# NickTravers/NeuralNetworkLibrary

Measured on AMD Instinct MI355X. Metric: ResNet-34 224x224 training throughput (Learner.train1minibatch, fwd+loss+bwd+optimizer), higher is better.
Workload: dtype f32; 1 GPU; DogsCats ResNet-34 classifier, 224x224, bs=64 per GPU, SGD momentum 0.9, fp32; global_batch=64, image_size=224, parallelism=dp1

## Files before the change

### include/nnl.h

```cpp
#ifndef NNL_H_
#define NNL_H_

#include <stddef.h>
#include <stdint.h>

#ifdef __cplusplus
extern "C" {
#endif

typedef enum {
  NNL_OK = 0,
  NNL_ERR_INVALID_ARG = -1,
  NNL_ERR_HIP = -2,
  NNL_ERR_UNSUPPORTED = -3,
  NNL_ERR_WORKSPACE = -4
} nnl_status_t;

int nnl_version(void);
const char* nnl_last_error(void);
int nnl_reload_env(void);

enum { NNL_PROF_CONV_FWD = 0, NNL_PROF_CONV_DGRAD = 1, NNL_PROF_CONV_WGRAD = 2, NNL_PROF_EMBDOT = 3,
       NNL_PROF_TABULAR = 4, NNL_PROF_RETINA_LOSS = 5, NNL_PROF_LSTM = 6, NNL_PROF_SOFTMAX_CE = 7,
       NNL_PROF_ELEMENTWISE = 8, NNL_PROF_GEMM = 9, NNL_PROF_OPTIM = 10, NNL_PROF_KINDS = 11 };
int nnl_prof_enable(int enable);
int nnl_prof_collect(int64_t* launches, double* total_ms, double* total_work);
int nnl_prof_collect2(int64_t* launches, double* total_ms, double* total_work, double* total_exec);
int nnl_dp_bump(int32_t* step, void* stream);
int nnl_dp_signal(int32_t* flag, const int32_t* step, void* stream);
int nnl_dp_wait(const int32_t* flag, int32_t value, int64_t timeout_us, int32_t* err, void* stream);
const char* nnl_source_stamp(void);

int nnl_embdotbias_fwd(const int64_t* x, const float* U, const float* M, const float* bu, const float* bi,
                       float* y, float* z, int64_t n, int64_t n_user, int64_t n_item, int64_t D,
                       int has_range, float lo, float hi, int32_t* err_flag, void* stream);
size_t nnl_embdotbias_bwd_workspace_bytes(int64_t n);
int nnl_embdotbias_bwd(const int64_t* x, const float* U, const float* M, const float* z, const float* dy,
                       float* dU, float* dM, float* dbu, float* dbi, int64_t n, int64_t n_user,
                       int64_t n_item, int64_t D, int has_range, float lo, float hi, void* workspace, size_t workspace_bytes, void* stream);

typedef struct {
  int32_t N, H, W, C;
  int32_t K, R, S;
  int32_t stride, pad;
  int32_t P, Q;
} nnl_conv_geom_t;

size_t nnl_conv2d_fwd_workspace_bytes(const nnl_conv_geom_t* g);
int64_t nnl_conv2d_tile_counters(void);
int nnl_conv2d_fwd(const float* x, const float* w, const float* bias, float* y, const nnl_conv_geom_t* g,
                   int relu, void* workspace, size_t workspace_bytes, int32_t* tile_counters, float* bn_partials,
                   const float* bn_pivot, int32_t* bn_rows, void* stream);
int nnl_conv2d_fwd_add_up2(const float* x, const float* w, const float* bias, const float* small, float* y,
                           const nnl_conv_geom_t* g, void* stream);
int nnl_upsample2_bwd(const float* dy, float* dsmall, int64_t N, int64_t h, int64_t w, int64_t C, void* stream);
int nnl_conv2d_weight_transpose(const float* w, float* wt, int K, int R, int S, int C, void* stream);
typedef struct {
  const float* w;
  float* wt;
  int32_t K, RS, C, first_tile;
} nnl_wt_desc_t;
int nnl_conv2d_weight_transpose_multi(const nnl_wt_desc_t* desc, const int32_t* tile_tensor, int64_t n_tiles,
                                      double total_elems, void* stream);
size_t nnl_conv2d_dgrad_workspace_bytes(const nnl_conv_geom_t* g);
int nnl_conv2d_dgrad(const float* dy, const float* wt, float* dx, const nnl_conv_geom_t* g, const float* addend,
                     void* workspace, size_t workspace_bytes, int32_t* tile_counters, void* stream);
typedef struct {
  const float* src;
  float* dst;
  int32_t rows, ch, flip, first_block;
  int32_t two_d, reserved;
} nnl_wino_desc_t;
int nnl_conv2d_wino_preferred(const nnl_conv_geom_t* g, int dgrad);
int nnl_wino_filter_multi(const nnl_wino_desc_t* desc, const int32_t* block_desc, int64_t n_blocks, void* stream);
int nnl_conv2d_fwd_pre(const float* x, const float* w, const float* bias, float* y, const nnl_conv_geom_t* g, int relu,
                       void* workspace, size_t workspace_bytes, int32_t* tile_counters, float* bn_partials, const float* bn_pivot,
                       int32_t* bn_rows, const float* u, void* stream);
int nnl_conv2d_dgrad_pre(const float* dy, const float* wt, float* dx, const nnl_conv_geom_t* g, const float* addend,
                         void* workspace, size_t workspace_bytes, int32_t* tile_counters, const float* u, void* stream);
size_t nnl_debug_conv_wino_workspace_bytes(int N, int H, int W, int C, int K);
int nnl_debug_conv_wino_fwd(const float* x, const float* filt, const float* bias, const float* add, float* y, void* ws,
                            size_t ws_bytes, int32_t* counters, long n_counters, float* bn_part, const float* bn_pivot, int N,
                            int H, int W, int C, int K, int relu, int flip, void* stream);
size_t nnl_debug_conv_wino2_workspace_bytes(int N, int H, int W, int C, int K);
int nnl_debug_conv_wino2_fwd(const float* x, const float* filt, const float* bias, const float* add, float* y, void* ws,
                            size_t ws_bytes, int32_t* counters, long n_counters, float* bn_part, const float* bn_pivot, int N,
                            int H, int W, int C, int K, int relu, int flip, void* stream);
int nnl_debug_conv_plan_times(int N, int H, int W, int C, int K, double* out);

int nnl_debug_route_record(int enable);
int nnl_debug_route_collect(char* out, size_t n);
size_t nnl_conv2d_wgrad_workspace_bytes(const nnl_conv_geom_t* g);
int nnl_conv2d_wgrad(const float* x, const float* dy, float* dw, const nnl_conv_geom_t* g, void* workspace,
                     size_t workspace_bytes, void* stream);
size_t nnl_colsum_workspace_bytes(int64_t rows, int64_t cols);
int nnl_sum_tensors(const float* const* src, int n, float* out, int64_t numel, void* stream);
int nnl_colsum(const float* a, float* out, int64_t rows, int64_t cols, void* workspace, size_t workspace_bytes,
               void* stream);
int nnl_relu_gate_colsum(const float* dy, const float* y, float* g, float* colsum, int64_t rows, int64_t cols, void* workspace,
                         size_t workspace_bytes, void* stream);
int nnl_act_gate_colsum(const float* dy, const float* y, float* g, float* colsum, int64_t rows, int64_t cols, int act,
                        void* workspace, size_t workspace_bytes, void* stream);

size_t nnl_bn_workspace_bytes(int64_t rows, int64_t C);
int nnl_bn_fwd(const float* x, const float* gamma, const float* beta, const float* residual, float* y,
               float* save_mean, float* save_invstd, float* running_mean, float* running_var, int64_t rows,
               int64_t C, float eps, float momentum, int training, int relu, int64_t* num_batches_tracked,
               uint32_t* relu_mask, const float* ext_partials, int64_t ext_rows, const float* ext_pivot, float* pivot_out,
               void* workspace, size_t workspace_bytes, void* stream);
int nnl_bn_bwd(const float* dy, const float* y, const uint32_t* relu_mask, const float* x, const float* gamma,
               const float* mean, const float* invstd, float* dx, float* dres, float* dgamma, float* dbeta, int64_t rows,
               int64_t C, int training, int relu, void* workspace, size_t workspace_bytes, void* stream);

int nnl_bn_relu_maxpool_supported(int64_t C);
int nnl_bn_relu_maxpool_fwd(const float* x, const float* gamma, const float* beta, float* y, uint8_t* idx, float* save_mean,
                            float* save_invstd, float* save_scale, float* save_shift, float* running_mean, float* running_var,
                            int64_t N, int64_t H, int64_t W, int64_t C, int64_t P, int64_t Q, int ks, int stride, int pad, float eps,
                            float momentum, int training, int64_t* num_batches_tracked, void* workspace, size_t workspace_bytes,
                            void* stream);
int nnl_bn_relu_maxpool_bwd(const float* dpool, const float* y, const uint8_t* idx, const float* x, const float* gamma,
                            const float* beta, const float* mean, const float* invstd, const float* scale, const float* shift,
                            float* dx, float* dgamma, float* dbeta,
                            int64_t N, int64_t H, int64_t W, int64_t C, int64_t P, int64_t Q, int ks, int stride, int pad,
                            int training, void* workspace, size_t workspace_bytes, void* stream);

int nnl_bn_sync_stats(const float* x, float* stats, int64_t rows, int64_t C, void* workspace, size_t workspace_bytes,
                      void* stream);
int nnl_bn_sync_fwd(const float* x, const float* all_stats, int world, const float* gamma, const float* beta,
                    const float* residual, float* y, float* save_mean, float* save_invstd, float* running_mean,
                    float* running_var, int64_t rows, int64_t C, float eps, float momentum, int relu,
                    int64_t* num_batches_tracked, uint32_t* relu_mask, void* workspace, size_t workspace_bytes, void* stream);
int nnl_bn_sync_bwd_reduce(const float* dy, const float* y, const uint32_t* relu_mask, const float* x, const float* mean,
                           const float* invstd, float* sums, int64_t rows, int64_t C, int relu, void* workspace,
                           size_t workspace_bytes, void* stream);
int nnl_bn_sync_bwd(const float* dy, const float* y, const uint32_t* relu_mask, const float* x, const float* gamma,
                    const float* mean, const float* invstd, const float* local_sums, const float* global_sums,
                    const float* all_stats,
                    int world, float* dx, float* dres, float* dgamma, float* dbeta, int64_t rows, int64_t C, int relu,
                    void* workspace, size_t workspace_bytes, void* stream);

int nnl_maxpool2d_fwd(const float* x, float* y, uint8_t* idx, int64_t N, int64_t H, int64_t W, int64_t C, int64_t P,
                      int64_t Q, int ksize, int stride, int pad, void* stream);
int nnl_maxpool2d_bwd(const float* dy, const uint8_t* idx, float* dx, int64_t N, int64_t H, int64_t W, int64_t C,
                      int64_t P, int64_t Q, int ksize, int stride, int pad, void* stream);
int nnl_concat_pool_fwd(const float* x, float* out, int32_t* argmax, int64_t N, int64_t HW, int64_t C, void* stream);
int nnl_concat_pool_bwd(const float* dout, const int32_t* argmax, float* dx, int64_t N, int64_t HW, int64_t C, void* stream);

int nnl_bbox_decode(const float* anchors, const float* reg, const float* clas, int64_t bs, int64_t A, int64_t K,
                    const float* mean4, const float* std4, float thresh, float width, float height, float* cand_boxes,
                    int32_t* cand_classes, float* cand_scores, int32_t* cand_order, int32_t* cand_count, void* stream);
size_t nnl_nms_workspace_bytes(int64_t bs, int64_t top_k);
int nnl_nms(const float* cand_boxes, const int32_t* cand_classes, const float* cand_scores, const int32_t* cand_order,
            const int32_t* cand_count, int64_t bs, int64_t cap, int64_t top_k, float max_overlap, float* kept_boxes,
            int32_t* kept_classes, float* kept_scores, int32_t* kept_count, void* workspace, size_t workspace_bytes,
            void* stream);

int nnl_tab_renorm(const int64_t* xcat, float* const* tables, const int32_t* card, const int32_t* dim,
                   const int32_t* row_off, const int32_t* row_table, int32_t* flags, int64_t bs, int32_t ncat,
                   int32_t total_rows, float max_norm, int32_t* err_flag, void* stream);
int nnl_tab_gather_fwd(const int64_t* xcat, const float* const* tables, const int32_t* card, const int32_t* dim,
                       const int32_t* col_off, const int32_t* col_table, const float* row_mask, const float* cont,
                       const float* cont_mask, float* out, int64_t bs, int32_t ncat, int32_t cat_width,
                       int32_t n_cont, int32_t ld_out, void* stream);
size_t nnl_tab_scatter_bwd_workspace_bytes(int64_t bs, int32_t ncat);
int nnl_tab_scatter_bwd(const int64_t* xcat, const int32_t* card, const int32_t* dim, const int32_t* col_off,
                        const int32_t* col_table, const int64_t* grad_off, const float* row_mask,
                        const float* cont_mask, const float* dout, float* dtab_flat, int64_t dtab_elems,
                        float* dcont, int64_t bs, int32_t ncat, int32_t cat_width, int32_t n_cont, int32_t ld_out,
                        void* workspace, size_t workspace_bytes, void* stream);
int nnl_tab_scan_bwd(const int64_t* xcat, const int32_t* card, const int32_t* dim, const int32_t* col_off,
                     const int64_t* grad_off, const float* row_mask, const float* cont_mask, const float* dout,
                     float* dtab_flat, float* dcont, const int32_t* blk_col, const int32_t* blk_first, int32_t n_scan_blocks,
                     int32_t max_dim, int64_t bs, int32_t ncat, int32_t cat_width, int32_t n_cont, int32_t ld_out, void* stream);

int nnl_pad_cols(const float* src, float* dst, int64_t rows, int64_t C, int64_t Cp, void* stream);
int nnl_keep_masks(const float* u, float* a, int64_t na, float keep_a, float* b, int64_t nb, float keep_b, void* stream);

int nnl_linear_small_supported(int64_t N);
int nnl_linear_small_fwd(const float* x, const float* w, const float* bias, float* y, int64_t M, int64_t K, int64_t ldx, int64_t N,
                         void* stream);
size_t nnl_linear_small_bwd_workspace_bytes(int64_t M, int64_t K, int64_t N);
int nnl_linear_small_bwd(const float* dy, const float* x, const float* w, float* dx, float* dw, float* db, int64_t M, int64_t K,
                         int64_t ldx, int64_t N, void* workspace, size_t workspace_bytes, void* stream);

size_t nnl_retina_loss_workspace_bytes(int64_t bs, int64_t A);
int nnl_retina_loss_fwd(const float* anchors, const float* reg, const float* clas, const float* boxes,
                        const int64_t* cats, int32_t* state, float* npos, float* out, int64_t bs, int64_t A,
                        int64_t K, int64_t M, float beta, float alpha, float gamma, void* workspace,
                        size_t workspace_bytes, void* stream);
int nnl_retina_loss_bwd(const float* anchors, const float* reg, const float* clas, const float* boxes,
                        const int64_t* cats, const int32_t* state, const float* npos, const float* grad_out,
                        float* dreg, float* dclas, int64_t bs, int64_t A, int64_t K, int64_t M, float beta,
                        float alpha, float gamma, void* stream);

int64_t nnl_lstm_padded_hidden(int64_t H);
int64_t nnl_lstm_padded_gates(int64_t H);
size_t nnl_lstm_workspace_bytes(int64_t T, int64_t B, int64_t H);
int nnl_lstm_fwd(const float* gx, const float* w_hh_pad, const float* h0, const float* c0, float* y, float* cy,
                 float* gates, int64_t T, int64_t B, int64_t H, void* workspace, size_t workspace_bytes, int32_t* err_flag,
                 void* stream);
int nnl_lstm_bwd(const float* dy, const float* dhT, const float* dcT, const float* gates, const float* cy,
                 const float* c0, const float* w_hh_t_pad, float* dgates_pad, float* dh0, float* dc0, int64_t T, int64_t B,
                 int64_t H, void* workspace, size_t workspace_bytes, int32_t* err_flag, void* stream);
int nnl_debug_lstm_bptt2_plan(int64_t B, int64_t H, int32_t* out5);

size_t nnl_mse_workspace_bytes(int64_t n);
int nnl_mse_fwd(const float* pred, const float* target, float* loss, int64_t n, void* workspace, size_t workspace_bytes, void* stream);
int nnl_mse_bwd(const float* pred, const float* target, const float* grad_out, float* dpred, int64_t n, void* stream);
int nnl_scaled_sigmoid_fwd(const float* x, float* y, float* sig, int64_t n, float lo, float hi, void* stream);
int nnl_scaled_sigmoid_bwd(const float* dy, const float* sig, float* dx, int64_t n, float lo, float hi, void* stream);

int nnl_embedding_rowmask_fwd(const int64_t* x, const float* W, const float* rowmask, float* out, int64_t n,
                              int64_t V, int64_t D, int32_t* err_flag, void* stream);
size_t nnl_embedding_rowmask_bwd_workspace_bytes(int64_t n);
int nnl_embedding_rowmask_bwd(const int64_t* x, const float* rowmask, const float* dout, float* dW, int64_t n,
                              int64_t V, int64_t D, int64_t padding_idx, void* workspace, size_t workspace_bytes, void* stream);
int nnl_softmax_ce_fwd(const float* logits, const int64_t* target, float* lse, float* loss_rows, float* loss_mean,
                       int64_t rows, int64_t V, int32_t* err_flag, void* stream);
int nnl_softmax_ce_bwd(const float* logits, const int64_t* target, const float* lse, const float* grad_out,
                       float* dlogits, int64_t rows, int64_t V, int64_t ld_dlogits, void* stream);
size_t nnl_seq_reg_workspace_bytes(int64_t T, int64_t R);
int nnl_seq_reg_fwd(const float* h, float* out3, int64_t T, int64_t R, float alpha, float beta, void* workspace,
                    size_t workspace_bytes, void* stream);
int nnl_seq_reg_bwd(const float* h, const float* grad_out, float* dh, int64_t T, int64_t R, float alpha, float beta, void* stream);
int nnl_weight_drop(const float* src, int64_t ld_src, const float* mask, float* out, int64_t ld_out, int64_t rows, int64_t H,
                    uint64_t seed, float p, void* stream);

size_t nnl_attn_pool_workspace_bytes(int64_t T, int64_t B, int64_t E, int64_t A);
int nnl_attn_pool_fwd(const float* h, const float* w2, const float* b2, const float* enc_out, const int64_t* x, int64_t pad_token,
                      float* attn, float* pooled, int64_t T, int64_t B, int64_t E, int64_t A, void* workspace, size_t workspace_bytes,
                      int32_t* counters, int64_t n_counters, void* stream);
int nnl_attn_pool_bwd(const float* h, const float* w2, const float* enc_out, const float* attn, const float* dpooled,
                      const float* dattn, float* dh, float* denc, float* dw2, float* db2, int64_t T, int64_t B, int64_t E, int64_t A,
                      void* workspace, size_t workspace_bytes, int32_t* counters, int64_t n_counters, void* stream);

typedef struct {
  float* param;
  float* grad;
  float* state1;
  float* state2;
  int64_t numel;
  float lr;
  float decay;
} nnl_optim_tensor_t;
int64_t nnl_optim_chunk_elems(void);
int nnl_optim_patch(nnl_optim_tensor_t* tensors, float* hyper, const float* dyn, int64_t n, void* stream);
int nnl_optim_step(const nnl_optim_tensor_t* tensors, const int32_t* chunk_tensor, const int64_t* chunk_off,
                   int64_t n_chunks, int kind, const float* hyper, int use_clip, float* clip_workspace, void* stream);

#ifdef __cplusplus
}
#endif
#endif
```

### neuralnetworklibrary_amd/_lib.py

```python
import ctypes as C
import os

import torch

_HERE = os.path.dirname(os.path.abspath(__file__))
LIB_PATH = os.environ.get('NNL_LIB_PATH') or os.path.join(_HERE, 'libnnl_hip.so')

if not os.path.exists(LIB_PATH):
    raise ImportError(
        f"{LIB_PATH} not found: build it with `python -c 'import __graft_entry__ as g; g.build()'` "
        "(or `make -C neuralnetworklibrary_amd/csrc`). There is no CPU fallback for the HIP hot path.")

lib = C.CDLL(LIB_PATH)

c_p = C.c_void_p
i32, i64, f32, f64 = C.c_int32, C.c_int64, C.c_float, C.c_double
sz = C.c_size_t


class ConvGeom(C.Structure):
    _fields_ = [('N', i32), ('H', i32), ('W', i32), ('C', i32), ('K', i32), ('R', i32), ('S', i32),
                ('stride', i32), ('pad', i32), ('P', i32), ('Q', i32)]


SIGNATURES = {
    'nnl_version': (C.c_int, []),
    'nnl_last_error': (C.c_char_p, []),
    'nnl_reload_env': (C.c_int, []),
    'nnl_prof_enable': (C.c_int, [C.c_int]),
    'nnl_prof_collect': (C.c_int, [C.POINTER(i64), C.POINTER(f64), C.POINTER(f64)]),
    'nnl_prof_collect2': (C.c_int, [C.POINTER(i64), C.POINTER(f64), C.POINTER(f64), C.POINTER(f64)]),
    'nnl_source_stamp': (C.c_char_p, []),
    'nnl_dp_bump': (C.c_int, [c_p, c_p]),
    'nnl_dp_signal': (C.c_int, [c_p, c_p, c_p]),
    'nnl_dp_wait': (C.c_int, [c_p, i32, i64, c_p, c_p]),
    'nnl_embdotbias_fwd': (C.c_int, [c_p, c_p, c_p, c_p, c_p, c_p, c_p, i64, i64, i64, i64, C.c_int, f32, f32,
                                     c_p, c_p]),
    'nnl_embdotbias_bwd_workspace_bytes': (sz, [i64]),
    'nnl_embdotbias_bwd': (C.c_int, [c_p, c_p, c_p, c_p, c_p, c_p, c_p, c_p, c_p, i64, i64, i64, i64, C.c_int,
                                     f32, f32, c_p, sz, c_p]),
    'nnl_conv2d_fwd_workspace_bytes': (sz, [C.POINTER(ConvGeom)]),
    'nnl_conv2d_dgrad_workspace_bytes': (sz, [C.POINTER(ConvGeom)]),
    'nnl_conv2d_tile_counters': (i64, []),
    'nnl_conv2d_wino_preferred': (C.c_int, [C.POINTER(ConvGeom), C.c_int]),
    'nnl_wino_filter_multi': (C.c_int, [c_p, c_p, i64, c_p]),
    'nnl_conv2d_fwd_pre': (C.c_int, [c_p, c_p, c_p, c_p, C.POINTER(ConvGeom), C.c_int, c_p, sz, c_p, c_p, c_p, C.POINTER(i32), c_p, c_p]),
    'nnl_conv2d_dgrad_pre': (C.c_int, [c_p, c_p, c_p, C.POINTER(ConvGeom), c_p, c_p, sz, c_p, c_p, c_p]),
    'nnl_debug_conv_wino_workspace_bytes': (sz, [C.c_int] * 5),
    'nnl_debug_conv_wino_fwd': (C.c_int, [c_p] * 6 + [sz, c_p, C.c_long, c_p, c_p] + [C.c_int] * 7 + [c_p]),
    'nnl_debug_conv_wino2_workspace_bytes': (sz, [C.c_int] * 5),
    'nnl_debug_conv_wino2_fwd': (C.c_int, [c_p] * 6 + [sz, c_p, C.c_long, c_p, c_p] + [C.c_int] * 7 + [c_p]),
    'nnl_debug_conv_plan_times': (C.c_int, [C.c_int] * 5 + [C.POINTER(C.c_double)]),
    'nnl_debug_route_record': (C.c_int, [C.c_int]),
    'nnl_debug_route_collect': (C.c_int, [C.c_char_p, sz]),
    'nnl_conv2d_fwd': (C.c_int, [c_p, c_p, c_p, c_p, C.POINTER(ConvGeom), C.c_int, c_p, sz, c_p, c_p, c_p, C.POINTER(i32), c_p]),
    'nnl_conv2d_weight_transpose': (C.c_int, [c_p, c_p, C.c_int, C.c_int, C.c_int, C.c_int, c_p]),
    'nnl_conv2d_weight_transpose_multi': (C.c_int, [c_p, c_p, i64, f64, c_p]),
    'nnl_conv2d_dgrad': (C.c_int, [c_p, c_p, c_p, C.POINTER(ConvGeom), c_p, c_p, sz, c_p, c_p]),
    'nnl_conv2d_wgrad_workspace_bytes': (sz, [C.POINTER(ConvGeom)]),
    'nnl_conv2d_wgrad': (C.c_int, [c_p, c_p, c_p, C.POINTER(ConvGeom), c_p, sz, c_p]),
    'nnl_colsum_workspace_bytes': (sz, [i64, i64]),
    'nnl_colsum': (C.c_int, [c_p, c_p, i64, i64, c_p, sz, c_p]),
    'nnl_relu_gate_colsum': (C.c_int, [c_p, c_p, c_p, c_p, i64, i64, c_p, sz, c_p]),
    'nnl_conv2d_fwd_add_up2': (C.c_int, [c_p, c_p, c_p, c_p, c_p, C.POINTER(ConvGeom), c_p]),
    'nnl_upsample2_bwd': (C.c_int, [c_p, c_p, i64, i64, i64, i64, c_p]),
    'nnl_act_gate_colsum': (C.c_int, [c_p, c_p, c_p, c_p, i64, i64, C.c_int, c_p, sz, c_p]),
    'nnl_maxpool2d_fwd': (C.c_int, [c_p, c_p, c_p, i64, i64, i64, i64, i64, i64, C.c_int, C.c_int, C.c_int, c_p]),
    'nnl_maxpool2d_bwd': (C.c_int, [c_p, c_p, c_p, i64, i64, i64, i64, i64, i64, C.c_int, C.c_int, C.c_int, c_p]),
    'nnl_sum_tensors': (C.c_int, [c_p, C.c_int, c_p, i64, c_p]),
    'nnl_bn_relu_maxpool_supported': (C.c_int, [i64]),
    'nnl_bn_relu_maxpool_fwd': (C.c_int, [c_p, c_p, c_p, c_p, c_p, c_p, c_p, c_p, c_p, c_p, c_p, i64, i64, i64, i64, i64, i64,
                                          C.c_int, C.c_int, C.c_int, f32, f32, C.c_int, c_p, c_p, sz, c_p]),
    'nnl_bn_relu_maxpool_bwd': (C.c_int, [c_p, c_p, c_p, c_p, c_p, c_p, c_p, c_p, c_p, c_p, c_p, c_p, c_p, i64, i64, i64, i64, i64, i64,
                                          C.c_int, C.c_int, C.c_int, C.c_int, c_p, sz, c_p]),
    'nnl_concat_pool_fwd': (C.c_int, [c_p, c_p, c_p, i64, i64, i64, c_p]),
    'nnl_concat_pool_bwd': (C.c_int, [c_p, c_p, c_p, i64, i64, i64, c_p]),
    'nnl_bbox_decode': (C.c_int, [c_p, c_p, c_p, i64, i64, i64, c_p, c_p, f32, f32, f32, c_p, c_p, c_p, c_p, c_p, c_p]),
    'nnl_nms_workspace_bytes': (sz, [i64, i64]),
    'nnl_nms': (C.c_int, [c_p, c_p, c_p, c_p, c_p, i64, i64, i64, f32, c_p, c_p, c_p, c_p, c_p, sz, c_p]),
    'nnl_tab_renorm': (C.c_int, [c_p, c_p, c_p, c_p, c_p, c_p, c_p, i64, i32, i32, f32, c_p, c_p]),
    'nnl_tab_gather_fwd': (C.c_int, [c_p, c_p, c_p, c_p, c_p, c_p, c_p, c_p, c_p, c_p, i64, i32, i32, i32, i32, c_p]),
    'nnl_tab_scatter_bwd_workspace_bytes': (sz, [i64, i32]),
    'nnl_tab_scatter_bwd': (C.c_int, [c_p, c_p, c_p, c_p, c_p, c_p, c_p, c_p, c_p, c_p, i64, c_p, i64, i32, i32, i32, i32, c_p, sz, c_p]),
    'nnl_tab_scan_bwd': (C.c_int, [c_p] * 12 + [i32, i32, i64, i32, i32, i32, i32, c_p]),
    'nnl_pad_cols': (C.c_int, [c_p, c_p, i64, i64, i64, c_p]),
    'nnl_keep_masks': (C.c_int, [c_p, c_p, i64, f32, c_p, i64, f32, c_p]),
    'nnl_linear_small_supported': (C.c_int, [i64]),
    'nnl_linear_small_fwd': (C.c_int, [c_p, c_p, c_p, c_p, i64, i64, i64, i64, c_p]),
    'nnl_linear_small_bwd_workspace_bytes': (sz, [i64, i64, i64]),
    'nnl_linear_small_bwd': (C.c_int, [c_p, c_p, c_p, c_p, c_p, c_p, i64, i64, i64, i64, c_p, sz, c_p]),
    'nnl_retina_loss_workspace_bytes': (sz, [i64, i64]),
    'nnl_retina_loss_fwd': (C.c_int, [c_p, c_p, c_p, c_p, c_p, c_p, c_p, c_p, i64, i64, i64, i64, f32, f32, f32, c_p, sz, c_p]),
    'nnl_retina_loss_bwd': (C.c_int, [c_p, c_p, c_p, c_p, c_p, c_p, c_p, c_p, c_p, c_p, i64, i64, i64, i64, f32, f32, f32, c_p]),
    'nnl_lstm_padded_hidden': (i64, [i64]),
    'nnl_lstm_padded_gates': (i64, [i64]),
    'nnl_lstm_workspace_bytes': (sz, [i64, i64, i64]),
    'nnl_lstm_fwd': (C.c_int, [c_p, c_p, c_p, c_p, c_p, c_p, c_p, i64, i64, i64, c_p, sz, c_p, c_p]),
    'nnl_lstm_bwd': (C.c_int, [c_p, c_p, c_p, c_p, c_p, c_p, c_p, c_p, c_p, c_p, i64, i64, i64, c_p, sz, c_p, c_p]),
    'nnl_debug_lstm_bptt2_plan': (C.c_int, [i64, i64, c_p]),
    'nnl_embedding_rowmask_fwd': (C.c_int, [c_p, c_p, c_p, c_p, i64, i64, i64, c_p, c_p]),
    'nnl_embedding_rowmask_bwd_workspace_bytes': (sz, [i64]),
    'nnl_embedding_rowmask_bwd': (C.c_int, [c_p, c_p, c_p, c_p, i64, i64, i64, i64, c_p, sz, c_p]),
    'nnl_softmax_ce_fwd': (C.c_int, [c_p, c_p, c_p, c_p, c_p, i64, i64, c_p, c_p]),
    'nnl_softmax_ce_bwd': (C.c_int, [c_p, c_p, c_p, c_p, c_p, i64, i64, i64, c_p]),
    'nnl_mse_workspace_bytes': (sz, [i64]),
    'nnl_mse_fwd': (C.c_int, [c_p, c_p, c_p, i64, c_p, sz, c_p]),
    'nnl_mse_bwd': (C.c_int, [c_p, c_p, c_p, c_p, i64, c_p]),
    'nnl_scaled_sigmoid_fwd': (C.c_int, [c_p, c_p, c_p, i64, C.c_float, C.c_float, c_p]),
    'nnl_scaled_sigmoid_bwd': (C.c_int, [c_p, c_p, c_p, i64, C.c_float, C.c_float, c_p]),
    'nnl_seq_reg_workspace_bytes': (sz, [i64, i64]),
    'nnl_seq_reg_fwd': (C.c_int, [c_p, c_p, i64, i64, C.c_float, C.c_float, c_p, sz, c_p]),
    'nnl_seq_reg_bwd': (C.c_int, [c_p, c_p, c_p, i64, i64, C.c_float, C.c_float, c_p]),
    'nnl_weight_drop': (C.c_int, [c_p, i64, c_p, c_p, i64, i64, i64, C.c_uint64, C.c_float, c_p]),
    'nnl_attn_pool_workspace_bytes': (sz, [i64, i64, i64, i64]),
    'nnl_attn_pool_fwd': (C.c_int, [c_p, c_p, c_p, c_p, c_p, i64, c_p, c_p, i64, i64, i64, i64, c_p, sz, c_p, i64, c_p]),
    'nnl_attn_pool_bwd': (C.c_int, [c_p, c_p, c_p, c_p, c_p, c_p, c_p, c_p, c_p, c_p, i64, i64, i64, i64, c_p, sz, c_p, i64, c_p]),
    'nnl_optim_chunk_elems': (i64, []),
    'nnl_optim_patch': (C.c_int, [c_p, c_p, c_p, i64, c_p]),
    'nnl_optim_step': (C.c_int, [c_p, c_p, c_p, i64, C.c_int, c_p, C.c_int, c_p, c_p]),
    'nnl_bn_workspace_bytes': (sz, [i64, i64]),
    'nnl_bn_fwd': (C.c_int, [c_p, c_p, c_p, c_p, c_p, c_p, c_p, c_p, c_p, i64, i64, f32, f32, C.c_int, C.c_int, c_p, c_p, c_p, i64,
                             c_p, c_p, c_p, sz, c_p]),
    'nnl_bn_sync_stats': (C.c_int, [c_p, c_p, i64, i64, c_p, sz, c_p]),
    'nnl_bn_sync_fwd': (C.c_int, [c_p, c_p, C.c_int, c_p, c_p, c_p, c_p, c_p, c_p, c_p, c_p, i64, i64, f32, f32, C.c_int, c_p,
                                  c_p, c_p, sz, c_p]),
    'nnl_bn_sync_bwd_reduce': (C.c_int, [c_p, c_p, c_p, c_p, c_p, c_p, c_p, i64, i64, C.c_int, c_p, sz, c_p]),
    'nnl_bn_sync_bwd': (C.c_int, [c_p, c_p, c_p, c_p, c_p, c_p, c_p, c_p, c_p, c_p, C.c_int, c_p, c_p, c_p, c_p, i64, i64,
                                  C.c_int, c_p, sz, c_p]),
    'nnl_bn_bwd': (C.c_int, [c_p, c_p, c_p, c_p, c_p, c_p, c_p, c_p, c_p, c_p, c_p, i64, i64, C.c_int, C.c_int, c_p, sz, c_p]),
}

for _name, (_res, _args) in SIGNATURES.items():
    try:
        _fn = getattr(lib, _name)
    except AttributeError as e:
        raise ImportError(f"libnnl_hip.so does not export {_name}; rebuild it") from e
    _fn.restype = _res
    _fn.argtypes = _args

PROF_KINDS = ['conv_fwd', 'conv_dgrad', 'conv_wgrad', 'embdot', 'tabular', 'retina_loss', 'lstm',
              'softmax_ce', 'elementwise', 'gemm', 'optim']


class NnlError(RuntimeError):
    pass


def check(status):
    if status != 0:
        raise NnlError(f"nnl error {status}: {lib.nnl_last_error().decode()}")


def ptr(t):
    return None if t is None else C.c_void_p(t.data_ptr())


def stream():
    return C.c_void_p(torch.cuda.current_stream().cuda_stream)


def require_cuda(*tensors):
    for t in tensors:
        if t is not None and not t.is_cuda:
            raise NnlError("nnl HIP op called with a non-CUDA tensor: the MI355X path has no CPU fallback")


def prof_enable(flag=True):
    check(lib.nnl_prof_enable(1 if flag else 0))


def prof_collect():
    n = len(PROF_KINDS)
    a, b, c, d = (i64 * n)(), (f64 * n)(), (f64 * n)(), (f64 * n)()
    check(lib.nnl_prof_collect2(a, b, c, d))
    return {k: {'launches': int(a[i]), 'ms': float(b[i]), 'work': float(c[i]), 'exec': float(d[i])} for i, k in enumerate(PROF_KINDS)}


def source_stamp_of_tree():
    import glob
    import hashlib
    csrc = os.path.join(os.path.dirname(os.path.abspath(__file__)), 'csrc')
    names = sorted(os.path.basename(p) for p in glob.glob(os.path.join(csrc, '*.hip')) + glob.glob(os.path.join(csrc, '*.h')))
    hsh = hashlib.sha256()
    for p in [os.path.join(csrc, n) for n in names] + [os.path.join(csrc, 'Makefile'), os.path.join(csrc, '..', '..', 'include', 'nnl.h')]:
        with open(p, 'rb') as f:
            hsh.update(f.read())
    return hsh.hexdigest()[:16]


def source_stamp():
    return lib.nnl_source_stamp().decode()
```

### neuralnetworklibrary_amd/csrc/batchnorm.hip

```cpp
#include "nnl_common.h"

namespace {

typedef float f32x4 __attribute__((ext_vector_type(4)));

template <int VEC> struct VecT;
template <> struct VecT<4> { typedef f32x4 type; };
template <> struct VecT<1> { typedef float type; };

template <int VEC> __device__ __forceinline__ float vget(const typename VecT<VEC>::type& v, int i);
template <> __device__ __forceinline__ float vget<4>(const f32x4& v, int i) { return v[i]; }
template <> __device__ __forceinline__ float vget<1>(const float& v, int i) { return v; }
template <int VEC> __device__ __forceinline__ void vset(typename VecT<VEC>::type& v, int i, float x);
template <> __device__ __forceinline__ void vset<4>(f32x4& v, int i, float x) { v[i] = x; }
template <> __device__ __forceinline__ void vset<1>(float& v, int i, float x) { v = x; }

constexpr int kBlock = 256;
constexpr int kMaxRowBlocks = 1024;
constexpr int kFinLanes = 64;

struct Shape {
  int L;
  int rpb;
  int gx, gy;
};

Shape make_shape(long rows, long CG) {
  Shape s;
  s.L = 1;
  while (s.L < 64 && s.L < CG) s.L <<= 1;
  s.rpb = kBlock / s.L;
  s.gy = (int)nnl_cdiv(CG, s.L);
  long gx = nnl_cdiv(rows, (long)s.rpb * 4);
  long cap = kMaxRowBlocks / (s.gy > 0 ? s.gy : 1);
  if (cap < 1) cap = 1;
  if (gx > cap) gx = cap;
  if (gx < 1) gx = 1;
  s.gx = (int)gx;
  return s;
}

template <int VEC>
__global__ __launch_bounds__(kBlock) void bn_stats_kernel(const float* __restrict__ x, float* __restrict__ part,
                                                           long rows, int C, int L) {
  typedef typename VecT<VEC>::type V;
  __shared__ float red[kBlock * 2 * VEC];
  const int CG = C / VEC;
  const int tx = threadIdx.x & (L - 1), ty = threadIdx.x / L;
  const int rpb = kBlock / L;
  const int g = blockIdx.y * L + tx;
  const bool ok = g < CG;
  float s1[VEC], s2[VEC], piv[VEC];
#pragma unroll
  for (int e = 0; e < VEC; ++e) { s1[e] = 0.f; s2[e] = 0.f; piv[e] = 0.f; }
  if (ok) {
    const V pv = *reinterpret_cast<const V*>(x + (long)g * VEC);
#pragma unroll
    for (int e = 0; e < VEC; ++e) piv[e] = vget<VEC>(pv, e);
    const long rstep = (long)gridDim.x * rpb;
    long r = (long)blockIdx.x * rpb + ty;
    const float* xp = x + (long)g * VEC;
    for (; r + 3 * rstep < rows; r += 4 * rstep) {
      V v[4];
#pragma unroll
      for (int u = 0; u < 4; ++u) v[u] = *reinterpret_cast<const V*>(xp + (r + u * rstep) * C);
#pragma unroll
      for (int u = 0; u < 4; ++u)
#pragma unroll
        for (int e = 0; e < VEC; ++e) {
          const float d = vget<VEC>(v[u], e) - piv[e];
          s1[e] += d;
          s2[e] += d * d;
        }
    }
    for (; r < rows; r += rstep) {
      const V v = *reinterpret_cast<const V*>(xp + r * C);
#pragma unroll
      for (int e = 0; e < VEC; ++e) {
        const float d = vget<VEC>(v, e) - piv[e];
        s1[e] += d;
        s2[e] += d * d;
      }
    }
  }
#pragma unroll
  for (int e = 0; e < VEC; ++e) {
    red[(threadIdx.x * VEC + e) * 2 + 0] = s1[e];
    red[(threadIdx.x * VEC + e) * 2 + 1] = s2[e];
  }
  __syncthreads();
  if (ty == 0 && ok) {
#pragma unroll
    for (int e = 0; e < VEC; ++e) {
      float a = 0.f, b = 0.f;
      for (int j = 0; j < rpb; ++j) {
        a += red[((j * L + tx) * VEC + e) * 2 + 0];
        b += red[((j * L + tx) * VEC + e) * 2 + 1];
      }
      const long c = (long)g * VEC + e;
      part[((long)blockIdx.x * C + c) * 2 + 0] = a;
      part[((long)blockIdx.x * C + c) * 2 + 1] = b;
    }
  }
}

template <int LANES = kFinLanes>
__device__ __forceinline__ void reduce_partials(const float* __restrict__ part, int nparts, int C, int c, bool cok,
                                                float (*red)[LANES][2], float& s1, float& s2) {
  const int lane = threadIdx.x & (LANES - 1), ch = threadIdx.x / LANES;
  float a = 0.f, b = 0.f;
  if (cok) {
    typedef float f32x2 __attribute__((ext_vector_type(2)));
    const f32x2* pp = reinterpret_cast<const f32x2*>(part) + c;
    int p = lane;
    constexpr int U = 8;
    for (; p + (U - 1) * LANES < nparts; p += U * LANES) {
      f32x2 v[U];
#pragma unroll
      for (int u = 0; u < U; ++u) v[u] = pp[(long)(p + u * LANES) * C];
#pragma unroll
      for (int u = 0; u < U; ++u) { a += v[u][0]; b += v[u][1]; }
    }
    for (; p < nparts; p += LANES) {
      const f32x2 v = pp[(long)p * C];
      a += v[0]; b += v[1];
    }
  }
  red[ch][lane][0] = a;
  red[ch][lane][1] = b;
  __syncthreads();
  for (int w = LANES / 2; w > 0; w >>= 1) {
    if (lane < w) {
      red[ch][lane][0] += red[ch][lane + w][0];
      red[ch][lane][1] += red[ch][lane + w][1];
    }
    __syncthreads();
  }
  s1 = red[ch][0][0];
  s2 = red[ch][0][1];
}

__device__ __forceinline__ void finish_stats(int c, int C, float m, float var, float n, const float* __restrict__ gamma,
                                             const float* __restrict__ beta, float* __restrict__ mean,
                                             float* __restrict__ invstd, float* __restrict__ running_mean,
                                             float* __restrict__ running_var, float* __restrict__ scale,
                                             float* __restrict__ shift, float eps, float momentum,
                                             float* __restrict__ pivot_out = nullptr) {
  const float is = 1.f / sqrtf(var + eps);
  mean[c] = m;
  if (pivot_out) pivot_out[c] = m;
  invstd[c] = is;
  if (running_mean) running_mean[c] = (1.f - momentum) * running_mean[c] + momentum * m;
  if (running_var) {
    const float unbiased = n > 1.f ? var * (n / (n - 1.f)) : var;
    running_var[c] = (1.f - momentum) * running_var[c] + momentum * unbiased;
  }
  const float gm = gamma ? gamma[c] : 1.f;
  const float sc = is * gm;
  scale[c] = sc;
  shift[c] = (beta ? beta[c] : 0.f) - m * sc;
}

template <int LANES>
__global__ void bn_finalize_kernel(const float* __restrict__ x, const float* __restrict__ part, int nparts,
                                   const float* __restrict__ gamma, const float* __restrict__ beta,
                                   float* __restrict__ mean, float* __restrict__ invstd,
                                   float* __restrict__ running_mean, float* __restrict__ running_var,
                                   float* __restrict__ scale, float* __restrict__ shift, long rows, int C, float eps,
                                   float momentum, long long* __restrict__ num_batches_tracked,
                                   float* __restrict__ pivot_out) {
  __shared__ float red[256 / LANES][LANES][2];
  const int c = blockIdx.x * (256 / LANES) + threadIdx.x / LANES;
  float s1, s2;
  reduce_partials<LANES>(part, nparts, C, c, c < C, red, s1, s2);
  if (c >= C || (threadIdx.x & (LANES - 1)) != 0) return;
  if (c == 0 && num_batches_tracked) *num_batches_tracked += 1;
  const float n = (float)rows;
  const float m = x[c] + s1 / n;
  float var = (s2 - s1 * (s1 / n)) / n;
  var = fmaxf(var, 0.f);
  finish_stats(c, C, m, var, n, gamma, beta, mean, invstd, running_mean, running_var, scale, shift, eps, momentum, pivot_out);
}

__global__ void bn_sync_local_kernel(const float* __restrict__ x, const float* __restrict__ part, int nparts,
                                     float* __restrict__ stats, long rows, int C) {
  __shared__ float red[4][kFinLanes][2];
  const int c = blockIdx.x * 4 + threadIdx.x / kFinLanes;
  float s1, s2;
  reduce_partials(part, nparts, C, c, c < C, red, s1, s2);
  if (c >= C || (threadIdx.x & (kFinLanes - 1)) != 0) return;
  const float n = (float)rows;
  stats[c] = x[c] + s1 / n;
  stats[C + c] = fmaxf(s2 - s1 * (s1 / n), 0.f);
  if (c == 0) {
    stats[2 * C] = (float)(rows >> 16);
    stats[2 * C + 1] = (float)(rows & 0xFFFF);
  }
}

__device__ __forceinline__ float sync_count(const float* __restrict__ st, int C) { return st[2 * C] * 65536.f + st[2 * C + 1]; }

__global__ void bn_sync_merge_kernel(const float* __restrict__ all_stats, int world, const float* __restrict__ gamma,
                                     const float* __restrict__ beta, float* __restrict__ mean, float* __restrict__ invstd,
                                     float* __restrict__ running_mean, float* __restrict__ running_var,
                                     float* __restrict__ scale, float* __restrict__ shift, int C, float eps, float momentum,
                                     long long* __restrict__ num_batches_tracked) {
  const int c = blockIdx.x * blockDim.x + threadIdx.x;
  if (c >= C) return;
  if (c == 0 && num_batches_tracked) *num_batches_tracked += 1;
  const long stride = 2L * C + 2;
  float n = 0.f, m = 0.f, M2 = 0.f;
  for (int r = 0; r < world; ++r) {
    const float* st = all_stats + r * stride;
    const float nr = sync_count(st, C);
    if (nr <= 0.f) continue;
    const float nn = n + nr;
    const float d = st[c] - m;
    m += d * (nr / nn);
    M2 += st[C + c] + d * d * (n * (nr / nn));
    n = nn;
  }
  finish_stats(c, C, m, fmaxf(M2 / n, 0.f), n, gamma, beta, mean, invstd, running_mean, running_var, scale, shift, eps, momentum);
}

__global__ void bn_eval_scale_kernel(const float* __restrict__ gamma, const float* __restrict__ beta,
                                     const float* __restrict__ running_mean, const float* __restrict__ running_var,
                                     float* __restrict__ scale, float* __restrict__ shift, float* __restrict__ invstd,
                                     int C, float eps) {
  const int c = blockIdx.x * blockDim.x + threadIdx.x;
  if (c >= C) return;
  const float is = 1.f / sqrtf(running_var[c] + eps);
  const float sc = is * (gamma ? gamma[c] : 1.f);
  scale[c] = sc;
  shift[c] = (beta ? beta[c] : 0.f) - running_mean[c] * sc;
  if (invstd) invstd[c] = is;
}

template <int VEC>
__device__ __forceinline__ unsigned keep_bits(const unsigned* __restrict__ mask, long i) {
  const long bit = i * VEC;
  return (mask[bit >> 5] >> (bit & 31)) & ((1u << VEC) - 1u);
}

template <int VEC>
__global__ __launch_bounds__(kBlock) void bn_apply_kernel(const float* __restrict__ x, const float* __restrict__ scale,
                                                           const float* __restrict__ shift,
                                                           const float* __restrict__ residual, float* __restrict__ y,
                                                           long total_v, int CG, int relu, unsigned* __restrict__ mask) {
  typedef typename VecT<VEC>::type V;
  const long stride = (long)gridDim.x * blockDim.x;
  const long i0 = (long)blockIdx.x * blockDim.x + threadIdx.x;
  const int lane = threadIdx.x & 63;
  const int g = (int)((unsigned long)i0 % (unsigned)CG);
  const V sc = reinterpret_cast<const V*>(scale)[g];
  const V sh = reinterpret_cast<const V*>(shift)[g];
  for (long base = i0 - lane; base < total_v; base += stride) {
    const long i = base + lane;
    const bool ok = i < total_v;
    unsigned bits = 0;
    if (ok) {
      const V xv = reinterpret_cast<const V*>(x)[i];
      V out;
      if (residual) {
        const V rv = reinterpret_cast<const V*>(residual)[i];
#pragma unroll
        for (int e = 0; e < VEC; ++e) vset<VEC>(out, e, vget<VEC>(xv, e) * vget<VEC>(sc, e) + vget<VEC>(sh, e) + vget<VEC>(rv, e));
      } else {
#pragma unroll
        for (int e = 0; e < VEC; ++e) vset<VEC>(out, e, vget<VEC>(xv, e) * vget<VEC>(sc, e) + vget<VEC>(sh, e));
      }
      if (relu) {
#pragma unroll
        for (int e = 0; e < VEC; ++e) {
          if (vget<VEC>(out, e) > 0.f) bits |= 1u << e;
          vset<VEC>(out, e, fmaxf(vget<VEC>(out, e), 0.f));
        }
      }
      reinterpret_cast<V*>(y)[i] = out;
    }
    if (mask != nullptr) {
      if (VEC == 4) {
        unsigned w = bits << ((lane & 7) * 4);
        w |= __shfl_xor(w, 1, 64);
        w |= __shfl_xor(w, 2, 64);
        w |= __shfl_xor(w, 4, 64);
        if ((lane & 7) == 0 && ok) mask[i >> 3] = w;
      } else {
        const unsigned long long b = __ballot(bits & 1u);
        if (lane == 0 && ok) mask[base >> 5] = (unsigned)b;
        if (lane == 32 && ok) mask[(base >> 5) + 1] = (unsigned)(b >> 32);
      }
    }
  }
}

template <int VEC>
__global__ __launch_bounds__(kBlock) void bn_bwd_reduce_kernel(const float* __restrict__ dy, const float* __restrict__ y,
                                                                const float* __restrict__ x, const float* __restrict__ mean,
                                                                const float* __restrict__ invstd, float* __restrict__ part,
                                                                long rows, int C, int L, int relu,
                                                                const unsigned* __restrict__ mask) {
  typedef typename VecT<VEC>::type V;
  __shared__ float red[kBlock * 2 * VEC];
  const int CG = C / VEC;
  const int tx = threadIdx.x & (L - 1), ty = threadIdx.x / L;
  const int rpb = kBlock / L;
  const int g = blockIdx.y * L + tx;
  const bool ok = g < CG;
  float s1[VEC], s2[VEC], mu[VEC], is[VEC];
#pragma unroll
  for (int e = 0; e < VEC; ++e) { s1[e] = 0.f; s2[e] = 0.f; mu[e] = 0.f; is[e] = 0.f; }
  if (ok) {
#pragma unroll
    for (int e = 0; e < VEC; ++e) { mu[e] = mean[(long)g * VEC + e]; is[e] = invstd[(long)g * VEC + e]; }
    const long rstep = (long)gridDim.x * rpb;
    long r = (long)blockIdx.x * rpb + ty;
    for (; r + rstep < rows; r += 2 * rstep) {
      V dv[2], xv[2], yv[2];
      unsigned kb[2] = {~0u, ~0u};
#pragma unroll
      for (int u = 0; u < 2; ++u) {
        const long off = (r + u * rstep) * C + (long)g * VEC;
        dv[u] = *reinterpret_cast<const V*>(dy + off);
        xv[u] = *reinterpret_cast<const V*>(x + off);
        yv[u] = dv[u];
        if (relu) {
          if (mask) kb[u] = keep_bits<VEC>(mask, off / VEC);
          else yv[u] = *reinterpret_cast<const V*>(y + off);
        }
      }
#pragma unroll
      for (int u = 0; u < 2; ++u)
#pragma unroll
        for (int e = 0; e < VEC; ++e) {
          float gg = vget<VEC>(dv[u], e);
          if (relu && (mask ? !((kb[u] >> e) & 1u) : !(vget<VEC>(yv[u], e) > 0.f))) gg = 0.f;
          s1[e] += gg;
          s2[e] += gg * ((vget<VEC>(xv[u], e) - mu[e]) * is[e]);
        }
    }
    for (; r < rows; r += rstep) {
      const long off = r * C + (long)g * VEC;
      const V dv = *reinterpret_cast<const V*>(dy + off);
      const V xv = *reinterpret_cast<const V*>(x + off);
      V yv = dv;
      unsigned kb = ~0u;
      if (relu) {
        if (mask) kb = keep_bits<VEC>(mask, off / VEC);
        else yv = *reinterpret_cast<const V*>(y + off);
      }
#pragma unroll
      for (int e = 0; e < VEC; ++e) {
        float gg = vget<VEC>(dv, e);
        if (relu && (mask ? !((kb >> e) & 1u) : !(vget<VEC>(yv, e) > 0.f))) gg = 0.f;
        s1[e] += gg;
        s2[e] += gg * ((vget<VEC>(xv, e) - mu[e]) * is[e]);
      }
    }
  }
#pragma unroll
  for (int e = 0; e < VEC; ++e) {
    red[(threadIdx.x * VEC + e) * 2 + 0] = s1[e];
    red[(threadIdx.x * VEC + e) * 2 + 1] = s2[e];
  }
  __syncthreads();
  if (ty == 0 && ok) {
#pragma unroll
    for (int e = 0; e < VEC; ++e) {
      float a = 0.f, b = 0.f;
      for (int j = 0; j < rpb; ++j) {
        a += red[((j * L + tx) * VEC + e) * 2 + 0];
        b += red[((j * L + tx) * VEC + e) * 2 + 1];
      }
      const long c = (long)g * VEC + e;
      part[((long)blockIdx.x * C + c) * 2 + 0] = a;
      part[((long)blockIdx.x * C + c) * 2 + 1] = b;
    }
  }
}

__global__ void bn_bwd_finalize_kernel(const float* __restrict__ part, int nparts, const float* __restrict__ gamma,
                                       const float* __restrict__ mean, const float* __restrict__ invstd,
                                       float* __restrict__ dgamma, float* __restrict__ dbeta, float* __restrict__ coef,
                                       long rows, int C, int training) {
  __shared__ float red[4][kFinLanes][2];
  const int c = blockIdx.x * 4 + threadIdx.x / kFinLanes;
  float s1, s2;
  reduce_partials(part, nparts, C, c, c < C, red, s1, s2);
  if (c >= C || (threadIdx.x & (kFinLanes - 1)) != 0) return;
  if (dbeta) dbeta[c] = s1;
  if (dgamma) dgamma[c] = s2;
  const float gm = gamma ? gamma[c] : 1.f;
  const float is = invstd[c], mu = mean[c];
  const float a = gm * is;
  if (training) {
    const float n = (float)rows;
    const float bq = -a * is * (s2 / n);
    coef[c] = a;
    coef[C + c] = bq;
    coef[2 * C + c] = -a * (s1 / n) - bq * mu;
  } else {
    coef[c] = a;
    coef[C + c] = 0.f;
    coef[2 * C + c] = 0.f;
  }
}

__global__ void bn_sync_bwd_sums_kernel(const float* __restrict__ part, int nparts, float* __restrict__ sums, int C) {
  __shared__ float red[4][kFinLanes][2];
  const int c = blockIdx.x * 4 + threadIdx.x / kFinLanes;
  float s1, s2;
  reduce_partials(part, nparts, C, c, c < C, red, s1, s2);
  if (c >= C || (threadIdx.x & (kFinLanes - 1)) != 0) return;
  sums[c] = s1;
  sums[C + c] = s2;
}

__global__ void bn_sync_bwd_coef_kernel(const float* __restrict__ local_sums, const float* __restrict__ global_sums,
                                        const float* __restrict__ all_stats, int world, const float* __restrict__ gamma,
                                        const float* __restrict__ mean, const float* __restrict__ invstd,
                                        float* __restrict__ dgamma, float* __restrict__ dbeta, float* __restrict__ coef, int C) {
  const int c = blockIdx.x * blockDim.x + threadIdx.x;
  if (c >= C) return;
  float n = 0.f;
  for (int r = 0; r < world; ++r) n += sync_count(all_stats + r * (2L * C + 2), C);
  if (dbeta) dbeta[c] = local_sums[c];
  if (dgamma) dgamma[c] = local_sums[C + c];
  const float s1 = global_sums[c], s2 = global_sums[C + c];
  const float is = invstd[c], mu = mean[c];
  const float a = (gamma ? gamma[c] : 1.f) * is;
  const float bq = -a * is * (s2 / n);
  coef[c] = a;
  coef[C + c] = bq;
  coef[2 * C + c] = -a * (s1 / n) - bq * mu;
}

template <int VEC>
__global__ __launch_bounds__(kBlock) void bn_bwd_apply_kernel(const float* __restrict__ dy, const float* __restrict__ y,
                                                               const float* __restrict__ x, const float* __restrict__ coef,
                                                               float* __restrict__ dx, float* __restrict__ dres,
                                                               long total_v, int CG, int C, int relu,
                                                               const unsigned* __restrict__ mask) {
  typedef typename VecT<VEC>::type V;
  const long stride = (long)gridDim.x * blockDim.x;
  const long i0 = (long)blockIdx.x * blockDim.x + threadIdx.x;
  const int g = (int)((unsigned)i0 % (unsigned)CG);
  const V ca = reinterpret_cast<const V*>(coef)[g];
  const V cb = reinterpret_cast<const V*>(coef + C)[g];
  const V cc = reinterpret_cast<const V*>(coef + 2 * C)[g];
  for (long i = i0; i < total_v; i += stride) {
    const V dv = reinterpret_cast<const V*>(dy)[i];
    const V xv = reinterpret_cast<const V*>(x)[i];
    V gv = dv;
    if (relu) {
      if (mask) {
        const unsigned kb = keep_bits<VEC>(mask, i);
#pragma unroll
        for (int e = 0; e < VEC; ++e)
          if (!((kb >> e) & 1u)) vset<VEC>(gv, e, 0.f);
      } else {
        const V yv = reinterpret_cast<const V*>(y)[i];
#pragma unroll
        for (int e = 0; e < VEC; ++e)
          if (!(vget<VEC>(yv, e) > 0.f)) vset<VEC>(gv, e, 0.f);
      }
    }
    V out;
#pragma unroll
    for (int e = 0; e < VEC; ++e)
      vset<VEC>(out, e, vget<VEC>(ca, e) * vget<VEC>(gv, e) + vget<VEC>(cb, e) * vget<VEC>(xv, e) + vget<VEC>(cc, e));
    reinterpret_cast<V*>(dx)[i] = out;
    if (dres) reinterpret_cast<V*>(dres)[i] = gv;
  }
}

long gcd_l(long a, long b) { while (b) { long t = a % b; a = b; b = t; } return a; }

int ew_grid(long total_v, long CG) {
  const long unit = CG / gcd_l(CG, kBlock);
  long b = nnl_cdiv(total_v, (long)kBlock * 2);
  if (b > 8192) b = 8192;
  b = nnl_cdiv(b, unit) * unit;
  if (b < unit) b = unit;
  return (int)b;
}

}

extern "C" size_t nnl_bn_workspace_bytes(int64_t rows, int64_t C) {
  if (rows <= 0 || C <= 0) return 0;
  return (size_t)((long)kMaxRowBlocks * C * 2 + 5 * C) * sizeof(float);
}

extern "C" int nnl_bn_fwd(const float* x, const float* gamma, const float* beta, const float* residual, float* y,
                          float* save_mean, float* save_invstd, float* running_mean, float* running_var, int64_t rows,
                          int64_t C, float eps, float momentum, int training, int relu, int64_t* num_batches_tracked,
                          uint32_t* relu_mask, const float* ext_partials, int64_t ext_rows, const float* ext_pivot,
                          float* pivot_out, void* workspace, size_t workspace_bytes, void* stream) {
  NNL_CHECK_ARG(rows > 0 && C > 0 && C < (1 << 24), "bn_fwd: bad sizes rows=%ld C=%ld", (long)rows, (long)C);
  NNL_CHECK_ARG(x && y && save_mean && save_invstd, "bn_fwd: null pointer");
  NNL_CHECK_ARG(training || (running_mean && running_var), "bn_fwd: eval mode needs running statistics");
  if (workspace == nullptr || workspace_bytes < nnl_bn_workspace_bytes(rows, C))
    return nnl_set_error(NNL_ERR_WORKSPACE, "bn_fwd: workspace too small");
  hipStream_t s = (hipStream_t)stream;
  float* part = (float*)workspace;
  float* scale = part + (long)kMaxRowBlocks * C * 2;
  float* shift = scale + C;
  const int VEC = (C % 4 == 0) ? 4 : 1;
  const long CG = C / VEC;
  NnlProfScope prof(NNL_PROF_ELEMENTWISE, s, (double)rows * C * (training ? 12.0 : 8.0) + (residual ? 4.0 * rows * C : 0.0));
  if (training && ext_partials != nullptr && ext_rows > 0 && ext_pivot != nullptr) {
    if (ext_rows >= 1024)
      hipLaunchKernelGGL(bn_finalize_kernel<256>, dim3((unsigned)C), dim3(256), 0, s, ext_pivot, ext_partials, (int)ext_rows, gamma, beta,
                         save_mean, save_invstd, running_mean, running_var, scale, shift, (long)rows, (int)C, eps, momentum,
                         (long long*)num_batches_tracked, pivot_out);
    else
      hipLaunchKernelGGL(bn_finalize_kernel<kFinLanes>, dim3((unsigned)nnl_cdiv(C, 4)), dim3(256), 0, s, ext_pivot, ext_partials,
                         (int)ext_rows, gamma, beta, save_mean, save_invstd, running_mean, running_var, scale, shift, (long)rows,
                         (int)C, eps, momentum, (long long*)num_batches_tracked, pivot_out);
    NNL_CHECK_LAUNCH();
  } else if (training) {
    const Shape sh = make_shape(rows, CG);
    if (VEC == 4)
      hipLaunchKernelGGL(bn_stats_kernel<4>, dim3(sh.gx, sh.gy), dim3(kBlock), 0, s, x, part, (long)rows, (int)C, sh.L);
    else
      hipLaunchKernelGGL(bn_stats_kernel<1>, dim3(sh.gx, sh.gy), dim3(kBlock), 0, s, x, part, (long)rows, (int)C, sh.L);
    NNL_CHECK_LAUNCH();
    hipLaunchKernelGGL(bn_finalize_kernel<kFinLanes>, dim3((unsigned)nnl_cdiv(C, 4)), dim3(256), 0, s, x, part, sh.gx, gamma, beta,
                       save_mean, save_invstd, running_mean, running_var, scale, shift, (long)rows, (int)C, eps, momentum,
                       (long long*)num_batches_tracked, pivot_out);
    NNL_CHECK_LAUNCH();
  } else {
    NNL_CHECK_HIP(hipMemcpyAsync(save_mean, running_mean, sizeof(float) * C, hipMemcpyDeviceToDevice, s));
    hipLaunchKernelGGL(bn_eval_scale_kernel, dim3((unsigned)nnl_cdiv(C, 256)), dim3(256), 0, s, gamma, beta, running_mean,
                       running_var, scale, shift, save_invstd, (int)C, eps);
    NNL_CHECK_LAUNCH();
  }
  const long total_v = rows * CG;
  if (VEC == 4)
    hipLaunchKernelGGL(bn_apply_kernel<4>, dim3(ew_grid(total_v, CG)), dim3(kBlock), 0, s, x, scale, shift, residual, y, total_v,
                       (int)CG, relu, relu ? relu_mask : nullptr);
  else
    hipLaunchKernelGGL(bn_apply_kernel<1>, dim3(ew_grid(total_v, CG)), dim3(kBlock), 0, s, x, scale, shift, residual, y, total_v,
                       (int)CG, relu, relu ? relu_mask : nullptr);
  NNL_CHECK_LAUNCH();
  return NNL_OK;
}

extern "C" int nnl_bn_bwd(const float* dy, const float* y, const uint32_t* relu_mask, const float* x, const float* gamma,
                          const float* mean, const float* invstd, float* dx, float* dres, float* dgamma, float* dbeta,
                          int64_t rows, int64_t C, int training, int relu, void* workspace, size_t workspace_bytes,
                          void* stream) {
  NNL_CHECK_ARG(rows > 0 && C > 0 && C < (1 << 24), "bn_bwd: bad sizes");
  NNL_CHECK_ARG(dy && x && mean && invstd && dx && (y || relu_mask || !relu), "bn_bwd: null pointer");
  if (workspace == nullptr || workspace_bytes < nnl_bn_workspace_bytes(rows, C))
    return nnl_set_error(NNL_ERR_WORKSPACE, "bn_bwd: workspace too small");
  hipStream_t s = (hipStream_t)stream;
  float* part = (float*)workspace;
  float* coef = part + (long)kMaxRowBlocks * C * 2 + 2 * C;
  const int VEC = (C % 4 == 0) ? 4 : 1;
  const long CG = C / VEC;
  const Shape sh = make_shape(rows, CG);
  NnlProfScope prof(NNL_PROF_ELEMENTWISE, s, (double)rows * C * (relu ? 28.0 : 20.0) + (dres ? 4.0 * rows * C : 0.0));
  if (VEC == 4)
    hipLaunchKernelGGL(bn_bwd_reduce_kernel<4>, dim3(sh.gx, sh.gy), dim3(kBlock), 0, s, dy, y, x, mean, invstd, part, (long)rows,
                       (int)C, sh.L, relu, relu_mask);
  else
    hipLaunchKernelGGL(bn_bwd_reduce_kernel<1>, dim3(sh.gx, sh.gy), dim3(kBlock), 0, s, dy, y, x, mean, invstd, part, (long)rows,
                       (int)C, sh.L, relu, relu_mask);
  NNL_CHECK_LAUNCH();
  hipLaunchKernelGGL(bn_bwd_finalize_kernel, dim3((unsigned)nnl_cdiv(C, 4)), dim3(256), 0, s, part, sh.gx, gamma, mean, invstd,
                     dgamma, dbeta, coef, (long)rows, (int)C, training);
  NNL_CHECK_LAUNCH();
  const long total_v = rows * CG;
  if (VEC == 4)
    hipLaunchKernelGGL(bn_bwd_apply_kernel<4>, dim3(ew_grid(total_v, CG)), dim3(kBlock), 0, s, dy, y, x, coef, dx, dres, total_v,
                       (int)CG, (int)C, relu, relu_mask);
  else
    hipLaunchKernelGGL(bn_bwd_apply_kernel<1>, dim3(ew_grid(total_v, CG)), dim3(kBlock), 0, s, dy, y, x, coef, dx, dres, total_v,
                       (int)CG, (int)C, relu, relu_mask);
  NNL_CHECK_LAUNCH();
  return NNL_OK;
}

namespace {

__device__ __forceinline__ f32x4 bnpool_affine(const f32x4& x, const f32x4& sc, const f32x4& sh) {
  f32x4 z;
#pragma unroll
  for (int e = 0; e < 4; ++e) z[e] = x[e] * sc[e] + sh[e];
  return z;
}

__global__ __launch_bounds__(kBlock) void bnpool_fwd_kernel(const float* __restrict__ x, const float* __restrict__ scale,
                                                            const float* __restrict__ shift, float* __restrict__ y,
                                                            uint8_t* __restrict__ idx, int N, int H, int W, int C4, int P, int Q,
                                                            int ks, int stride, int pad) {
  const long total = (long)N * P * Q * C4;
  const long i0 = (long)blockIdx.x * blockDim.x + threadIdx.x;
  const int c4 = (int)(i0 % C4);
  const f32x4 sc = reinterpret_cast<const f32x4*>(scale)[c4], sh = reinterpret_cast<const f32x4*>(shift)[c4];
  for (long i = i0; i < total; i += (long)gridDim.x * blockDim.x) {
    long r = i / C4;
    const int q = (int)(r % Q); r /= Q;
    const int p = (int)(r % P);
    const int n = (int)(r / P);
    f32x4 best = {0.f, 0.f, 0.f, 0.f};
    int bi[4] = {-1, -1, -1, -1};
    for (int kh = 0; kh < ks; ++kh) {
      const int h = p * stride - pad + kh;
      if ((unsigned)h >= (unsigned)H) continue;
      for (int kw = 0; kw < ks; ++kw) {
        const int w = q * stride - pad + kw;
        if ((unsigned)w >= (unsigned)W) continue;
        f32x4 v = bnpool_affine(reinterpret_cast<const f32x4*>(x)[((long)(n * H + h) * W + w) * C4 + c4], sc, sh);
        const int t = kh * ks + kw;
#pragma unroll
        for (int e = 0; e < 4; ++e) {
          v[e] = (v[e] != v[e]) ? v[e] : fmaxf(v[e], 0.f);
          if (bi[e] < 0 || v[e] > best[e] || v[e] != v[e]) { best[e] = v[e]; bi[e] = t; }
        }
      }
    }
    reinterpret_cast<f32x4*>(y)[i] = best;
    reinterpret_cast<uchar4*>(idx)[i] = make_uchar4((uint8_t)bi[0], (uint8_t)bi[1], (uint8_t)bi[2], (uint8_t)bi[3]);
  }
}

struct PoolGeom { int H, W, C4, P, Q, ks, stride, pad; };

__device__ __forceinline__ f32x4 bnpool_grad(const float* __restrict__ dpool, const uint8_t* __restrict__ idx, const f32x4& xv,
                                             const f32x4& sc, const f32x4& sh, int n, int h, int w, int c4, const PoolGeom& g) {
  f32x4 acc = {0.f, 0.f, 0.f, 0.f};
  int p_lo = h + g.pad - g.ks + 1; p_lo = p_lo > 0 ? (p_lo + g.stride - 1) / g.stride : 0;
  int p_hi = (h + g.pad) / g.stride; if (p_hi > g.P - 1) p_hi = g.P - 1;
  int q_lo = w + g.pad - g.ks + 1; q_lo = q_lo > 0 ? (q_lo + g.stride - 1) / g.stride : 0;
  int q_hi = (w + g.pad) / g.stride; if (q_hi > g.Q - 1) q_hi = g.Q - 1;
  for (int p = p_lo; p <= p_hi; ++p) {
    const int kh = h + g.pad - p * g.stride;
    for (int q = q_lo; q <= q_hi; ++q) {
      const int t = kh * g.ks + (w + g.pad - q * g.stride);
      const long o = ((long)(n * g.P + p) * g.Q + q) * g.C4 + c4;
      const uchar4 id = reinterpret_cast<const uchar4*>(idx)[o];
      const f32x4 d = reinterpret_cast<const f32x4*>(dpool)[o];
      if (id.x == t) acc[0] += d[0];
      if (id.y == t) acc[1] += d[1];
      if (id.z == t) acc[2] += d[2];
      if (id.w == t) acc[3] += d[3];
    }
  }
  const f32x4 z = bnpool_affine(xv, sc, sh);
#pragma unroll
  for (int e = 0; e < 4; ++e) if (!(z[e] > 0.f)) acc[e] = 0.f;
  return acc;
}

constexpr int kPoolRedBlock = 1024;

__global__ __launch_bounds__(kPoolRedBlock) void bnpool_bwd_reduce_kernel(const float* __restrict__ dpool, const uint8_t* __restrict__ idx,
                                                                   const float* __restrict__ x, const float* __restrict__ scale,
                                                                   const float* __restrict__ shift, const float* __restrict__ mean,
                                                                   const float* __restrict__ invstd, float* __restrict__ part,
                                                                   int N, int C, PoolGeom g) {
  __shared__ float red[kPoolRedBlock][8];
  const long total = (long)N * g.H * g.W * g.C4;
  const long i0 = (long)blockIdx.x * blockDim.x + threadIdx.x;
  const int c4 = (int)(i0 % g.C4);
  const f32x4 sc = reinterpret_cast<const f32x4*>(scale)[c4], sh = reinterpret_cast<const f32x4*>(shift)[c4];
  const f32x4 mu = reinterpret_cast<const f32x4*>(mean)[c4], is = reinterpret_cast<const f32x4*>(invstd)[c4];
  float s1[4] = {0.f, 0.f, 0.f, 0.f}, s2[4] = {0.f, 0.f, 0.f, 0.f};
  for (long i = i0; i < total; i += (long)gridDim.x * blockDim.x) {
    long r = i / g.C4;
    const int w = (int)(r % g.W); r /= g.W;
    const int h = (int)(r % g.H);
    const int n = (int)(r / g.H);
    const f32x4 xv = reinterpret_cast<const f32x4*>(x)[i];
    const f32x4 gg = bnpool_grad(dpool, idx, xv, sc, sh, n, h, w, c4, g);
#pragma unroll
    for (int e = 0; e < 4; ++e) { s1[e] += gg[e]; s2[e] += gg[e] * ((xv[e] - mu[e]) * is[e]); }
  }
#pragma unroll
  for (int e = 0; e < 4; ++e) { red[threadIdx.x][e * 2] = s1[e]; red[threadIdx.x][e * 2 + 1] = s2[e]; }
  __syncthreads();
  if ((int)threadIdx.x < g.C4) {
#pragma unroll
    for (int e = 0; e < 4; ++e) {
      float a = 0.f, b = 0.f;
      for (int j = threadIdx.x; j < kPoolRedBlock; j += g.C4) { a += red[j][e * 2]; b += red[j][e * 2 + 1]; }
      const long c = (long)threadIdx.x * 4 + e;
      part[((long)blockIdx.x * C + c) * 2 + 0] = a;
      part[((long)blockIdx.x * C + c) * 2 + 1] = b;
    }
  }
}

__global__ __launch_bounds__(kPoolRedBlock) void bnpool_bwd_reduce_out_kernel(const float* __restrict__ dpool, const float* __restrict__ y,
                                                                       const uint8_t* __restrict__ idx, const float* __restrict__ x,
                                                                       const float* __restrict__ gamma, const float* __restrict__ beta,
                                                                       const float* __restrict__ mean, const float* __restrict__ invstd,
                                                                       float* __restrict__ part, int N, int C, PoolGeom g) {
  __shared__ float red[kPoolRedBlock][8];
  const long total = (long)N * g.P * g.Q * g.C4;
  const long i0 = (long)blockIdx.x * blockDim.x + threadIdx.x;
  const int c4 = (int)(i0 % g.C4);
  float bt[4], rg[4], mu[4], is[4];
  bool fast[4];
#pragma unroll
  for (int e = 0; e < 4; ++e) {
    const int c = c4 * 4 + e;
    const float gm = gamma ? gamma[c] : 1.f;
    bt[e] = beta ? beta[c] : 0.f;
    fast[e] = fabsf(gm) > 1e-2f;
    rg[e] = fast[e] ? 1.f / gm : 0.f;
    mu[e] = mean[c]; is[e] = invstd[c];
  }
  float s1[4] = {0.f, 0.f, 0.f, 0.f}, s2[4] = {0.f, 0.f, 0.f, 0.f};
  for (long i = i0; i < total; i += (long)gridDim.x * blockDim.x) {
    const f32x4 d = reinterpret_cast<const f32x4*>(dpool)[i];
    const f32x4 yv = reinterpret_cast<const f32x4*>(y)[i];
    const uchar4 id = reinterpret_cast<const uchar4*>(idx)[i];
    const unsigned char t[4] = {id.x, id.y, id.z, id.w};
#pragma unroll
    for (int e = 0; e < 4; ++e) {
      if (!(yv[e] > 0.f)) continue;
      float xh;
      if (fast[e]) {
        xh = (yv[e] - bt[e]) * rg[e];
      } else {
        long r = i / g.C4;
        const int q = (int)(r % g.Q); r /= g.Q;
        const int p = (int)(r % g.P);
        const int n = (int)(r / g.P);
        const int h = p * g.stride - g.pad + t[e] / g.ks, w = q * g.stride - g.pad + t[e] % g.ks;
        xh = (x[((long)(n * g.H + h) * g.W + w) * C + c4 * 4 + e] - mu[e]) * is[e];
      }
      s1[e] += d[e];
      s2[e] += d[e] * xh;
    }
  }
#pragma unroll
  for (int e = 0; e < 4; ++e) { red[threadIdx.x][e * 2] = s1[e]; red[threadIdx.x][e * 2 + 1] = s2[e]; }
  __syncthreads();
  if ((int)threadIdx.x < g.C4) {
#pragma unroll
    for (int e = 0; e < 4; ++e) {
      float a = 0.f, b = 0.f;
      for (int j = threadIdx.x; j < kPoolRedBlock; j += g.C4) { a += red[j][e * 2]; b += red[j][e * 2 + 1]; }
      const long c = (long)threadIdx.x * 4 + e;
      part[((long)blockIdx.x * C + c) * 2 + 0] = a;
      part[((long)blockIdx.x * C + c) * 2 + 1] = b;
    }
  }
}

__global__ __launch_bounds__(kBlock) void bnpool_bwd_apply_kernel(const float* __restrict__ dpool, const uint8_t* __restrict__ idx,
                                                                  const float* __restrict__ x, const float* __restrict__ scale,
                                                                  const float* __restrict__ shift, const float* __restrict__ coef,
                                                                  float* __restrict__ dx, int N, int C, PoolGeom g) {
  const long total = (long)N * g.H * g.W * g.C4;
  const long i0 = (long)blockIdx.x * blockDim.x + threadIdx.x;
  const int c4 = (int)(i0 % g.C4);
  const f32x4 sc = reinterpret_cast<const f32x4*>(scale)[c4], sh = reinterpret_cast<const f32x4*>(shift)[c4];
  const f32x4 ca = reinterpret_cast<const f32x4*>(coef)[c4], cb = *reinterpret_cast<const f32x4*>(coef + C + c4 * 4),
              cc = *reinterpret_cast<const f32x4*>(coef + 2 * C + c4 * 4);
  for (long i = i0; i < total; i += (long)gridDim.x * blockDim.x) {
    long r = i / g.C4;
    const int w = (int)(r % g.W); r /= g.W;
    const int h = (int)(r % g.H);
    const int n = (int)(r / g.H);
    const f32x4 xv = reinterpret_cast<const f32x4*>(x)[i];
    const f32x4 gg = bnpool_grad(dpool, idx, xv, sc, sh, n, h, w, c4, g);
    f32x4 out;
#pragma unroll
    for (int e = 0; e < 4; ++e) out[e] = ca[e] * gg[e] + cb[e] * xv[e] + cc[e];
    reinterpret_cast<f32x4*>(dx)[i] = out;
  }
}

bool bnpool_ok(long C) { return C % 4 == 0 && C >= 4 && C <= 1024 && (kBlock % (C / 4)) == 0; }
unsigned bnpool_grid(long total) {
  long g = nnl_cdiv(total, (long)kPoolRedBlock * 4);
  if (g > kMaxRowBlocks) g = kMaxRowBlocks;
  return (unsigned)(g < 1 ? 1 : g);
}

}

extern "C" int nnl_bn_relu_maxpool_supported(int64_t C) { return bnpool_ok(C) ? 1 : 0; }

extern "C" int nnl_bn_relu_maxpool_fwd(const float* x, const float* gamma, const float* beta, float* y, uint8_t* idx,
                                       float* save_mean, float* save_invstd, float* save_scale, float* save_shift,
                                       float* running_mean, float* running_var, int64_t N, int64_t H, int64_t W, int64_t C,
                                       int64_t P, int64_t Q, int ks, int stride, int pad, float eps, float momentum, int training,
                                       int64_t* num_batches_tracked, void* workspace, size_t workspace_bytes, void* stream) {
  const long rows = (long)N * H * W;
  NNL_CHECK_ARG(N > 0 && H > 0 && W > 0 && P > 0 && Q > 0 && ks > 0 && ks * ks <= 255 && stride > 0 && pad >= 0 && 2 * pad <= ks,
                "bn_relu_maxpool_fwd: bad geometry");
  NNL_CHECK_ARG(P == (H + 2 * pad - ks) / stride + 1 && Q == (W + 2 * pad - ks) / stride + 1, "bn_relu_maxpool_fwd: P/Q do not match");
  NNL_CHECK_ARG(bnpool_ok(C), "bn_relu_maxpool_fwd: C=%ld needs C %% 4 == 0 and C/4 dividing 256", (long)C);
  NNL_CHECK_ARG(x && y && idx && save_mean && save_invstd && save_scale && save_shift, "bn_relu_maxpool_fwd: null pointer");
  NNL_CHECK_ARG(training || (running_mean && running_var), "bn_relu_maxpool_fwd: eval mode needs running statistics");
  NNL_CHECK_ARG(rows * C < (1L << 31) * 4, "bn_relu_maxpool_fwd: tensor too large");
  if (workspace == nullptr || workspace_bytes < nnl_bn_workspace_bytes(rows, C))
    return nnl_set_error(NNL_ERR_WORKSPACE, "bn_relu_maxpool_fwd: workspace too small");
  hipStream_t s = (hipStream_t)stream;
  float* part = (float*)workspace;
  float* scale = save_scale;
  float* shift = save_shift;
  const long CG = C / 4;
  NnlProfScope prof(NNL_PROF_ELEMENTWISE, s, (double)rows * C * (training ? 8.0 : 4.0) + (double)N * P * Q * C * 5.0);
  if (training) {
    const Shape sh = make_shape(rows, CG);
    hipLaunchKernelGGL(bn_stats_kernel<4>, dim3(sh.gx, sh.gy), dim3(kBlock), 0, s, x, part, rows, (int)C, sh.L);
    NNL_CHECK_LAUNCH();
    hipLaunchKernelGGL(bn_finalize_kernel<kFinLanes>, dim3((unsigned)nnl_cdiv(C, 4)), dim3(256), 0, s, x, part, sh.gx, gamma, beta,
                       save_mean, save_invstd, running_mean, running_var, scale, shift, rows, (int)C, eps, momentum,
                       (long long*)num_batches_tracked, (float*)nullptr);
    NNL_CHECK_LAUNCH();
  } else {
    NNL_CHECK_HIP(hipMemcpyAsync(save_mean, running_mean, sizeof(float) * C, hipMemcpyDeviceToDevice, s));
    hipLaunchKernelGGL(bn_eval_scale_kernel, dim3((unsigned)nnl_cdiv(C, 256)), dim3(256), 0, s, gamma, beta, running_mean,
                       running_var, scale, shift, save_invstd, (int)C, eps);
    NNL_CHECK_LAUNCH();
  }
  const long total = (long)N * P * Q * CG;
  hipLaunchKernelGGL(bnpool_fwd_kernel, dim3((unsigned)nnl_cdiv(total, kBlock)), dim3(kBlock), 0, s, x, scale, shift, y, idx, (int)N,
                     (int)H, (int)W, (int)CG, (int)P, (int)Q, ks, stride, pad);
  NNL_CHECK_LAUNCH();
  return NNL_OK;
}

extern "C" int nnl_bn_relu_maxpool_bwd(const float* dpool, const float* y, const uint8_t* idx, const float* x, const float* gamma,
                                       const float* beta, const float* mean, const float* invstd, const float* scale,
                                       const float* shift, float* dx, float* dgamma, float* dbeta, int64_t N,
                                       int64_t H, int64_t W, int64_t C, int64_t P, int64_t Q, int ks, int stride, int pad,
                                       int training, void* workspace, size_t workspace_bytes, void* stream) {
  const long rows = (long)N * H * W;
  NNL_CHECK_ARG(N > 0 && H > 0 && W > 0 && P > 0 && Q > 0 && ks > 0 && stride > 0 && pad >= 0, "bn_relu_maxpool_bwd: bad geometry");
  NNL_CHECK_ARG(bnpool_ok(C), "bn_relu_maxpool_bwd: C=%ld needs C %% 4 == 0 and C/4 dividing 256", (long)C);
  NNL_CHECK_ARG(dpool && idx && x && mean && invstd && scale && shift && dx, "bn_relu_maxpool_bwd: null pointer");
  if (workspace == nullptr || workspace_bytes < nnl_bn_workspace_bytes(rows, C))
    return nnl_set_error(NNL_ERR_WORKSPACE, "bn_relu_maxpool_bwd: workspace too small");
  hipStream_t s = (hipStream_t)stream;
  float* part = (float*)workspace;
  float* coef = part + (long)kMaxRowBlocks * C * 2 + 2 * C;
  const PoolGeom g{(int)H, (int)W, (int)(C / 4), (int)P, (int)Q, ks, stride, pad};
  const long total = rows * (C / 4);
  const unsigned grid = bnpool_grid(total);
  NnlProfScope prof(NNL_PROF_ELEMENTWISE, s, (double)rows * C * 12.0 + (double)N * P * Q * C * 10.0);
  if (y != nullptr) {
    const unsigned go = bnpool_grid((long)N * P * Q * (C / 4));
    hipLaunchKernelGGL(bnpool_bwd_reduce_out_kernel, dim3(go), dim3(kPoolRedBlock), 0, s, dpool, y, idx, x, gamma, beta, mean, invstd,
                       part, (int)N, (int)C, g);
    NNL_CHECK_LAUNCH();
    hipLaunchKernelGGL(bn_bwd_finalize_kernel, dim3((unsigned)nnl_cdiv(C, 4)), dim3(256), 0, s, part, (int)go, gamma, mean, invstd,
                       dgamma, dbeta, coef, rows, (int)C, training);
    NNL_CHECK_LAUNCH();
  } else {
    hipLaunchKernelGGL(bnpool_bwd_reduce_kernel, dim3(grid), dim3(kPoolRedBlock), 0, s, dpool, idx, x, scale, shift, mean, invstd, part,
                       (int)N, (int)C, g);
    NNL_CHECK_LAUNCH();
    hipLaunchKernelGGL(bn_bwd_finalize_kernel, dim3((unsigned)nnl_cdiv(C, 4)), dim3(256), 0, s, part, (int)grid, gamma, mean, invstd,
                       dgamma, dbeta, coef, rows, (int)C, training);
    NNL_CHECK_LAUNCH();
  }
  hipLaunchKernelGGL(bnpool_bwd_apply_kernel, dim3((unsigned)nnl_cdiv(total, kBlock)), dim3(kBlock), 0, s, dpool, idx, x, scale, shift, coef, dx, (int)N, (int)C, g);
  NNL_CHECK_LAUNCH();
  return NNL_OK;
}

namespace {
int launch_stats(const float* x, float* part, long rows, long C, hipStream_t s, Shape& sh) {
  const int VEC = (C % 4 == 0) ? 4 : 1;
  sh = make_shape(rows, C / VEC);
  if (VEC == 4)
    hipLaunchKernelGGL(bn_stats_kernel<4>, dim3(sh.gx, sh.gy), dim3(kBlock), 0, s, x, part, rows, (int)C, sh.L);
  else
    hipLaunchKernelGGL(bn_stats_kernel<1>, dim3(sh.gx, sh.gy), dim3(kBlock), 0, s, x, part, rows, (int)C, sh.L);
  NNL_CHECK_LAUNCH();
  return NNL_OK;
}
}

extern "C" int nnl_bn_sync_stats(const float* x, float* stats, int64_t rows, int64_t C, void* workspace,
                                 size_t workspace_bytes, void* stream) {
  NNL_CHECK_ARG(rows > 0 && C > 0 && C < (1 << 24) && x && stats, "bn_sync_stats: bad arguments");
  if (workspace == nullptr || workspace_bytes < nnl_bn_workspace_bytes(rows, C))
    return nnl_set_error(NNL_ERR_WORKSPACE, "bn_sync_stats: workspace too small");
  hipStream_t s = (hipStream_t)stream;
  NnlProfScope prof(NNL_PROF_ELEMENTWISE, s, (double)rows * C * 4.0);
  Shape sh;
  int rc = launch_stats(x, (float*)workspace, rows, C, s, sh);
  if (rc != NNL_OK) return rc;
  hipLaunchKernelGGL(bn_sync_local_kernel, dim3((unsigned)nnl_cdiv(C, 4)), dim3(256), 0, s, x, (const float*)workspace, sh.gx,
                     stats, (long)rows, (int)C);
  NNL_CHECK_LAUNCH();
  return NNL_OK;
}

extern "C" int nnl_bn_sync_fwd(const float* x, const float* all_stats, int world, const float* gamma, const float* beta,
                               const float* residual, float* y, float* save_mean, float* save_invstd, float* running_mean,
                               float* running_var, int64_t rows, int64_t C, float eps, float momentum, int relu,
                               int64_t* num_batches_tracked, uint32_t* relu_mask, void* workspace, size_t workspace_bytes,
                               void* stream) {
  NNL_CHECK_ARG(rows > 0 && C > 0 && C < (1 << 24) && world > 0, "bn_sync_fwd: bad sizes");
  NNL_CHECK_ARG(x && y && all_stats && save_mean && save_invstd, "bn_sync_fwd: null pointer");
  if (workspace == nullptr || workspace_bytes < nnl_bn_workspace_bytes(rows, C))
    return nnl_set_error(NNL_ERR_WORKSPACE, "bn_sync_fwd: workspace too small");
  hipStream_t s = (hipStream_t)stream;
  float* scale = (float*)workspace + (long)kMaxRowBlocks * C * 2;
  float* shift = scale + C;
  NnlProfScope prof(NNL_PROF_ELEMENTWISE, s, (double)rows * C * 8.0 + (residual ? 4.0 * rows * C : 0.0));
  hipLaunchKernelGGL(bn_sync_merge_kernel, dim3((unsigned)nnl_cdiv(C, 256)), dim3(256), 0, s, all_stats, world, gamma, beta,
                     save_mean, save_invstd, running_mean, running_var, scale, shift, (int)C, eps, momentum,
                     (long long*)num_batches_tracked);
  NNL_CHECK_LAUNCH();
  const int VEC = (C % 4 == 0) ? 4 : 1;
  const long CG = C / VEC, total_v = rows * CG;
  if (VEC == 4)
    hipLaunchKernelGGL(bn_apply_kernel<4>, dim3(ew_grid(total_v, CG)), dim3(kBlock), 0, s, x, scale, shift, residual, y, total_v,
                       (int)CG, relu, relu ? relu_mask : nullptr);
  else
    hipLaunchKernelGGL(bn_apply_kernel<1>, dim3(ew_grid(total_v, CG)), dim3(kBlock), 0, s, x, scale, shift, residual, y, total_v,
                       (int)CG, relu, relu ? relu_mask : nullptr);
  NNL_CHECK_LAUNCH();
  return NNL_OK;
}

extern "C" int nnl_bn_sync_bwd_reduce(const float* dy, const float* y, const uint32_t* relu_mask, const float* x,
                                      const float* mean, const float* invstd, float* sums, int64_t rows, int64_t C, int relu,
                                      void* workspace, size_t workspace_bytes, void* stream) {
  NNL_CHECK_ARG(rows > 0 && C > 0 && C < (1 << 24), "bn_sync_bwd_reduce: bad sizes");
  NNL_CHECK_ARG(dy && x && mean && invstd && sums && (y || relu_mask || !relu), "bn_sync_bwd_reduce: null pointer");
  if (workspace == nullptr || workspace_bytes < nnl_bn_workspace_bytes(rows, C))
    return nnl_set_error(NNL_ERR_WORKSPACE, "bn_sync_bwd_reduce: workspace too small");
  hipStream_t s = (hipStream_t)stream;
  float* part = (float*)workspace;
  const int VEC = (C % 4 == 0) ? 4 : 1;
  const Shape sh = make_shape(rows, C / VEC);
  NnlProfScope prof(NNL_PROF_ELEMENTWISE, s, (double)rows * C * (relu ? 12.0 : 8.0));
  if (VEC == 4)
    hipLaunchKernelGGL(bn_bwd_reduce_kernel<4>, dim3(sh.gx, sh.gy), dim3(kBlock), 0, s, dy, y, x, mean, invstd, part, (long)rows,
                       (int)C, sh.L, relu, relu_mask);
  else
    hipLaunchKernelGGL(bn_bwd_reduce_kernel<1>, dim3(sh.gx, sh.gy), dim3(kBlock), 0, s, dy, y, x, mean, invstd, part, (long)rows,
                       (int)C, sh.L, relu, relu_mask);
  NNL_CHECK_LAUNCH();
  hipLaunchKernelGGL(bn_sync_bwd_sums_kernel, dim3((unsigned)nnl_cdiv(C, 4)), dim3(256), 0, s, (const float*)part, sh.gx, sums,
                     (int)C);
  NNL_CHECK_LAUNCH();
  return NNL_OK;
}

extern "C" int nnl_bn_sync_bwd(const float* dy, const float* y, const uint32_t* relu_mask, const float* x, const float* gamma,
                               const float* mean,
                               const float* invstd, const float* local_sums, const float* global_sums, const float* all_stats,
                               int world, float* dx, float* dres, float* dgamma, float* dbeta, int64_t rows, int64_t C, int relu,
                               void* workspace, size_t workspace_bytes, void* stream) {
  NNL_CHECK_ARG(rows > 0 && C > 0 && C < (1 << 24) && world > 0, "bn_sync_bwd: bad sizes");
  NNL_CHECK_ARG(dy && x && mean && invstd && dx && local_sums && global_sums && all_stats && (y || relu_mask || !relu),
                "bn_sync_bwd: null pointer");
  if (workspace == nullptr || workspace_bytes < nnl_bn_workspace_bytes(rows, C))
    return nnl_set_error(NNL_ERR_WORKSPACE, "bn_sync_bwd: workspace too small");
  hipStream_t s = (hipStream_t)stream;
  float* coef = (float*)workspace + (long)kMaxRowBlocks * C * 2 + 2 * C;
  NnlProfScope prof(NNL_PROF_ELEMENTWISE, s, (double)rows * C * (relu ? 16.0 : 12.0) + (dres ? 4.0 * rows * C : 0.0));
  hipLaunchKernelGGL(bn_sync_bwd_coef_kernel, dim3((unsigned)nnl_cdiv(C, 256)), dim3(256), 0, s, local_sums, global_sums, all_stats,
                     world, gamma, mean, invstd, dgamma, dbeta, coef, (int)C);
  NNL_CHECK_LAUNCH();
  const int VEC = (C % 4 == 0) ? 4 : 1;
  const long CG = C / VEC, total_v = rows * CG;
  if (VEC == 4)
    hipLaunchKernelGGL(bn_bwd_apply_kernel<4>, dim3(ew_grid(total_v, CG)), dim3(kBlock), 0, s, dy, y, x, coef, dx, dres, total_v,
                       (int)CG, (int)C, relu, relu_mask);
  else
    hipLaunchKernelGGL(bn_bwd_apply_kernel<1>, dim3(ew_grid(total_v, CG)), dim3(kBlock), 0, s, dy, y, x, coef, dx, dres, total_v,
                       (int)CG, (int)C, relu, relu_mask);
  NNL_CHECK_LAUNCH();
  return NNL_OK;
}
```

### neuralnetworklibrary_amd/ops.py

```python
import collections
import ctypes
import os
import weakref

import numpy as np
import torch

from . import _lib
from ._lib import check, lib, ptr, require_cuda, stream

__all__ = ['mse_loss', 'scaled_sigmoid', 'embdotbias', 'index_error_flag', 'raise_if_index_error', 'conv2d', 'to_nhwc', 'from_nhwc', 'linear', 'bn_act', 'concat_pool2d', 'TabularPlan', 'tab_embed_concat', 'embedding_renorm_drop', 'retina_loss']

_ERR_FLAGS = {}


def _flags(device):
    key = (device.type, device.index)
    if key not in _ERR_FLAGS:
        _ERR_FLAGS[key] = torch.zeros(2, dtype=torch.int32, device=device)
    return _ERR_FLAGS[key]


def index_error_flag(device):
    return _flags(device)[0:1]


def lstm_timeout_flag(device):
    return _flags(device)[1:2]


def raise_for_flag(code):
    if code & 2:
        raise _lib.NnlError("the persistent LSTM kernel's grid barrier timed out (results of that step are invalid)")
    if code & 1:
        raise IndexError("index out of range in self")


def raise_if_index_error():
    for flag in _ERR_FLAGS.values():
        v = flag.tolist()
        code = (1 if v[0] else 0) | (2 if v[1] else 0)
        if code:
            flag.zero_()
            raise_for_flag(code)


def _f32c(t):
    return t.contiguous() if t.dtype == torch.float32 else t.float().contiguous()


def _workspace(nbytes, device, *, floor=False):
    if not nbytes and not floor:
        return None
    return torch.empty(max((nbytes + 3) // 4, 1), dtype=torch.float32, device=device)


class _EmbDotBias(torch.autograd.Function):

    @staticmethod
    def forward(ctx, x, U, M, bu, bi, lo, hi):
        require_cuda(x, U, M, bu, bi)
        x = x.contiguous()
        if x.dtype != torch.int64:
            x = x.long()
        U, M, bu, bi = _f32c(U), _f32c(M), _f32c(bu), _f32c(bi)
        n, D = x.shape[0], U.shape[1]
        y = torch.empty(n, dtype=torch.float32, device=x.device)
        z = torch.empty(n, dtype=torch.float32, device=x.device)
        has_range = lo is not None
        check(lib.nnl_embdotbias_fwd(ptr(x), ptr(U), ptr(M), ptr(bu), ptr(bi), ptr(y), ptr(z), n, U.shape[0],
                                     M.shape[0], D, int(has_range), float(lo or 0.), float(hi or 0.),
                                     ptr(index_error_flag(x.device)), stream()))
        ctx.save_for_backward(x, U, M, z)
        ctx.rng = (has_range, float(lo or 0.), float(hi or 0.))
        return y

    @staticmethod
    def backward(ctx, dy):
        x, U, M, z = ctx.saved_tensors
        has_range, lo, hi = ctx.rng
        dy = _f32c(dy)
        nu, ni, D = U.shape[0], M.shape[0], U.shape[1]
        flat = torch.empty((nu + ni) * (D + 1), dtype=torch.float32, device=U.device)
        dU, dM = flat[:nu * D].view(nu, D), flat[nu * D:(nu + ni) * D].view(ni, D)
        dbu, dbi = flat[(nu + ni) * D:(nu + ni) * D + nu].view(nu, 1), flat[(nu + ni) * D + nu:].view(ni, 1)
        wsb = int(lib.nnl_embdotbias_bwd_workspace_bytes(x.shape[0]))
        ws = _workspace(wsb, U.device, floor=True)
        check(lib.nnl_embdotbias_bwd(ptr(x), ptr(U), ptr(M), ptr(z), ptr(dy), ptr(dU), ptr(dM), ptr(dbu), ptr(dbi),
                                     x.shape[0], U.shape[0], M.shape[0], U.shape[1], int(has_range), lo, hi,
                                     ptr(ws), wsb, stream()))
        return None, dU, dM, dbu, dbi, None, None


class _MSE(torch.autograd.Function):

    @staticmethod
    def forward(ctx, pred, target):
        require_cuda(pred, target)
        p, t = _f32c(pred).reshape(-1), _f32c(target).reshape(-1)
        n = p.numel()
        loss = torch.empty((), dtype=torch.float32, device=p.device)
        wsb = int(lib.nnl_mse_workspace_bytes(n))
        ws = _workspace(wsb, p.device)
        check(lib.nnl_mse_fwd(ptr(p), ptr(t), ptr(loss), n, ptr(ws), wsb, stream()))
        ctx.save_for_backward(p, t)
        ctx.shape = pred.shape
        return loss

    @staticmethod
    def backward(ctx, dloss):
        p, t = ctx.saved_tensors
        g = _f32c(dloss).reshape(1)
        dp = torch.empty_like(p)
        check(lib.nnl_mse_bwd(ptr(p), ptr(t), ptr(g), ptr(dp), p.numel(), stream()))
        return dp.view(ctx.shape), None


def mse_loss(pred, target):
    return _MSE.apply(pred, target)


class _ScaledSigmoid(torch.autograd.Function):

    @staticmethod
    def forward(ctx, x, lo, hi):
        require_cuda(x)
        xc = _f32c(x)
        y, sg = torch.empty_like(xc), torch.empty_like(xc)
        check(lib.nnl_scaled_sigmoid_fwd(ptr(xc), ptr(y), ptr(sg), xc.numel(), float(lo), float(hi), stream()))
        ctx.save_for_backward(sg)
        ctx.rng = (float(lo), float(hi))
        return y

    @staticmethod
    def backward(ctx, dy):
        sg, = ctx.saved_tensors
        dyc = _f32c(dy)
        dx = torch.empty_like(sg)
        check(lib.nnl_scaled_sigmoid_bwd(ptr(dyc), ptr(sg), ptr(dx), sg.numel(), ctx.rng[0], ctx.rng[1], stream()))
        return dx, None, None


def scaled_sigmoid(x, lo, hi):
    return _ScaledSigmoid.apply(x, float(lo), float(hi))


def embdotbias(x, U, M, bu, bi, output_range=None):
    lo, hi = (None, None) if output_range is None else (float(output_range[0]), float(output_range[1]))
    return _EmbDotBias.apply(x, U, M, bu, bi, lo, hi)


def to_nhwc(x):
    return x.permute(0, 2, 3, 1).contiguous()


def from_nhwc(x):
    return x.permute(0, 3, 1, 2)


def _geom(N, H, W, C, K, R, S, stride, pad):
    P = (H + 2 * pad - R) // stride + 1
    Q = (W + 2 * pad - S) // stride + 1
    return _lib.ConvGeom(N, H, W, C, K, R, S, stride, pad, P, Q)


def _pad_c4(t_nhwc):
    C = t_nhwc.shape[-1]
    if C % 4 == 0:
        return t_nhwc
    if t_nhwc.is_cuda and t_nhwc.dtype == torch.float32 and t_nhwc.is_contiguous() and not (torch.is_grad_enabled() and t_nhwc.requires_grad):
        Cp = C + 4 - C % 4
        out = torch.empty(t_nhwc.shape[:-1] + (Cp,), dtype=torch.float32, device=t_nhwc.device)
        check(lib.nnl_pad_cols(ptr(t_nhwc), ptr(out), t_nhwc.numel() // C, C, Cp, stream()))
        return out
    return torch.nn.functional.pad(t_nhwc, (0, 4 - C % 4))


_WT_ACTIVE = {}
_WT_PADDED = {}


_WINO_U_FWD, _WINO_U_BWD = {}, {}
_WINO_GEN = [0]
_WINO_IN_STEP = [False]
_WINO_PREF = {}


class _WinoBatch:

    def __init__(self, items):
        dev = items[0][1].device
        self.key = _wino_batch_key(items)
        total = sum(_wino_u_numel(t.shape[0], t.shape[3], mode) for _, t, _, mode in items)
        self.flat = torch.empty(total, dtype=torch.float32, device=dev)
        desc = np.zeros(len(items), dtype=np.dtype([('src', '<u8'), ('dst', '<u8'), ('rows', '<i4'), ('ch', '<i4'), ('flip', '<i4'), ('first', '<i4'),
                                                    ('two_d', '<i4'), ('reserved', '<i4')]))
        block_desc, self.views, off, first = [], {}, 0, 0
        for i, (k, t, flip, mode) in enumerate(items):
            rows, ch = t.shape[0], t.shape[3]
            n = _wino_u_numel(rows, ch, mode)
            u = self.flat[off:off + n]
            off += n
            nb = (rows * ch + 255) // 256 if mode == 2 else (rows * 3 * ch + 255) // 256
            desc[i] = (t.data_ptr(), u.data_ptr(), rows, ch, flip, first, 1 if mode == 2 else 0, 0)
            block_desc += [i] * nb
            first += nb
            self.views[(k, mode)] = u
        self.n_blocks = first
        self.desc = torch.from_numpy(desc.view(np.uint8).copy()).to(dev)
        self.block_desc = torch.tensor(block_desc, dtype=torch.int32, device=dev)

    def run(self):
        check(lib.nnl_wino_filter_multi(ptr(self.desc), ptr(self.block_desc), self.n_blocks, stream()))


def _wino_u_numel(rows, ch, mode):
    return rows * 16 * ch if mode == 2 else rows * 12 * ch


def _wino_batch_key(items):
    return tuple((k, t.data_ptr(), tuple(t.shape), mode) for k, t, _, mode in items)


def _conv_mods(model):
    mods = getattr(model, '_nnl_conv_mods', None)
    if mods is None:
        mods = [m for m in model.modules() if getattr(m, 'nnl_hip_conv', False)]
        object.__setattr__(model, '_nnl_conv_mods', mods)
    return mods


def prepared_batches(model):
    return tuple(b for b in (getattr(model, a, None) for a in ('_nnl_wino_fwd_batch', '_nnl_wino_bwd_batch', '_nnl_wt_batch')) if b is not None)


def _run_wino_batch(model, attr, items, out):
    if not items:
        return
    key = _wino_batch_key(items)
    batch = getattr(model, attr, None)
    if batch is None or batch.key != key:
        if torch.cuda.is_current_stream_capturing():
            return
        batch = _WinoBatch(items)
        object.__setattr__(model, attr, batch)
    batch.run()
    out.update(batch.views)


def _wino_modes(key_ptr, which):
    e = _WINO_PREF.get(key_ptr)
    return e[which][1] if e is not None else ()


def prepare_forward(model):
    _WINO_U_FWD.clear()
    _WINO_GEN[0] += 1
    _WINO_IN_STEP[0] = True
    if os.environ.get('NNL_WINO_PREPARE', '1') == '0':
        return
    items = []
    for m in _conv_mods(model):
        w = m.weight
        modes = _wino_modes(w.data_ptr(), 0)
        if (modes and w.is_cuda and w.dim() == 4 and w.shape[2] == 3 and w.shape[3] == 3 and w.dtype == torch.float32
                and w.is_contiguous(memory_format=torch.channels_last)):
            for mode in sorted(modes):
                items.append((w.data_ptr(), w.permute(0, 2, 3, 1), 0, mode))
    _run_wino_batch(model, '_nnl_wino_fwd_batch', items, _WINO_U_FWD)


class _WtBatch:

    def __init__(self, weights):
        dev = weights[0].device
        self.key = tuple((w.data_ptr(), tuple(w.shape)) for w in weights)
        total = sum(w.numel() for w in weights)
        self.flat = torch.empty(total, dtype=torch.float32, device=dev)
        desc = np.zeros(len(weights), dtype=np.dtype([('w', '<u8'), ('wt', '<u8'), ('K', '<i4'), ('RS', '<i4'), ('C', '<i4'), ('first', '<i4')]))
        tile_tensor, self.views, off, first = [], {}, 0, 0
        for i, w in enumerate(weights):
            K, C, R, S = w.shape
            wt = self.flat[off:off + w.numel()].view(C, R, S, K)
            off += w.numel()
            n_tiles = R * S * ((K + 31) // 32) * ((C + 31) // 32)
            desc[i] = (w.data_ptr(), wt.data_ptr(), K, R * S, C, first)
            tile_tensor += [i] * n_tiles
            first += n_tiles
            self.views[w.data_ptr()] = wt
        self.n_tiles, self.total = first, float(total)
        self.desc = torch.from_numpy(desc.view(np.uint8).copy()).to(dev)
        self.tile_tensor = torch.tensor(tile_tensor, dtype=torch.int32, device=dev)

    def run(self):
        check(lib.nnl_conv2d_weight_transpose_multi(ptr(self.desc), ptr(self.tile_tensor), self.n_tiles, self.total, stream()))


def prepare_backward(model):
    mods = _conv_mods(model)
    ws = [m.weight for m in mods
          if m.weight.is_cuda and m.weight.dim() == 4 and m.weight.shape[1] % 4 == 0
          and m.weight.shape[0] % 4 == 0 and m.weight.dtype == torch.float32
          and m.weight.is_contiguous(memory_format=torch.channels_last)]
    if len(ws) < 2 or sum(w.requires_grad for w in ws) * 2 < len(ws):
        return
    key = tuple((w.data_ptr(), tuple(w.shape)) for w in ws)
    batch = getattr(model, '_nnl_wt_batch', None)
    if batch is None or batch.key != key:
        if torch.cuda.is_current_stream_capturing():
            return
        batch = _WtBatch(ws)
        object.__setattr__(model, '_nnl_wt_batch', batch)
    batch.run()
    _WT_ACTIVE.clear()
    _WT_ACTIVE.update(batch.views)
    _WINO_U_BWD.clear()
    if os.environ.get('NNL_WINO_PREPARE', '1') != '0':
        items = [(w.data_ptr(), batch.views[w.data_ptr()], 1, mode) for w in ws if w.shape[2] == 3 and w.shape[3] == 3
                 for mode in sorted(_wino_modes(w.data_ptr(), 1))]
        _run_wino_batch(model, '_nnl_wino_bwd_batch', items, _WINO_U_BWD)


def finish_backward():
    _WT_ACTIVE.clear()
    _WT_PADDED.clear()
    _WINO_U_FWD.clear()
    _WINO_U_BWD.clear()
    _WINO_IN_STEP[0] = False


def _wino_pref(key_ptr, which, g):
    pref = int(lib.nnl_conv2d_wino_preferred(g, which)) if (g.R == 3 and g.S == 3 and g.stride == 1) else 0
    if (pref or key_ptr in _WINO_PREF) and (which == 1 or _WINO_IN_STEP[0]):
        if len(_WINO_PREF) > 8192:
            _WINO_PREF.clear()
        e = _WINO_PREF.setdefault(key_ptr, [[-1, set()], [-1, set()]])[which]
        if e[0] != _WINO_GEN[0]:
            e[0], e[1] = _WINO_GEN[0], set()
        if pref:
            e[1].add(pref)
    return pref


_PADDED_GRADS = {}


def register_padded_grad(base, ld):
    if len(_PADDED_GRADS) > 64:
        for k in [k for k, (r, _) in _PADDED_GRADS.items() if r() is None]:
            del _PADDED_GRADS[k]
    _PADDED_GRADS[id(base)] = (weakref.ref(base), int(ld))


def _padded_rows(dy, K):
    base = dy._base if dy._is_view() else None
    ent = _PADDED_GRADS.get(id(base)) if base is not None else None
    if ent is None or ent[0]() is not base or dy.dim() != 4 or dy.shape[2] != 1 or dy.shape[3] != 1:
        return None
    ld = ent[1]
    if dy.dtype != torch.float32 or dy.stride(1) != 1 or dy.stride(0) != ld or ld < K or ld % 16 != 0 or dy.storage_offset() % ld != 0:
        return None
    if dy.storage_offset() + dy.shape[0] * ld > base.numel():
        return None
    return torch.as_strided(base, (dy.shape[0], 1, 1, ld), (ld, ld, ld, 1), dy.storage_offset())


_TILE_COUNTERS = {}


def _tile_counters(device):
    t = _TILE_COUNTERS.get(device.index)
    if t is None:
        if torch.cuda.is_current_stream_capturing():
            return None
        t = _TILE_COUNTERS[device.index] = torch.zeros(int(lib.nnl_conv2d_tile_counters()), dtype=torch.int32, device=device)
    return t


class GradSlot:
    __slots__ = ('tensor', 'closed')

    def __init__(self):
        self.tensor = None
        self.closed = False



_FAN = {}


class _FanOut(torch.autograd.Function):
    @staticmethod
    def forward(ctx, p, n):
        ctx.n = n
        return tuple(p.detach().view(p.shape) for _ in range(n))

    @staticmethod
    def backward(ctx, *grads):
        have = [g for g in grads if g is not None]
        if not have:
            return None, None
        if len(have) == 1:
            return have[0], None
        g0 = have[0]
        dense = all(g.is_cuda and g.dtype == torch.float32 and g.shape == g0.shape and g.stride() == g0.stride() and g.data_ptr() % 16 == 0
                    and (g.is_contiguous() or (g.dim() == 4 and g.is_contiguous(memory_format=torch.channels_last))) for g in have)
        if not dense or len(have) > 8:
            out = have[0]
            for g in have[1:]:
                out = out + g
            return out, None
        out = torch.empty_like(g0)
        arr = (ctypes.c_void_p * len(have))(*[g.data_ptr() for g in have])
        check(lib.nnl_sum_tensors(arr, len(have), ptr(out), g0.numel(), stream()))
        return out, None


class shared_params:

    def __init__(self, modules, n):
        self.modules, self.n, self.keys = modules, int(n), []

    def __enter__(self):
        if self.n > 1 and torch.is_grad_enabled():
            for m in self.modules:
                for p in m.parameters():
                    if p.requires_grad and p.is_cuda and id(p) not in _FAN:
                        _FAN[id(p)] = list(_FanOut.apply(p, self.n))
                        self.keys.append(id(p))
        return self

    def __exit__(self, *exc):
        for k in self.keys:
            _FAN.pop(k, None)
        return False


def fan_param(p):
    if p is None or not _FAN:
        return p
    lst = _FAN.get(id(p))
    return lst.pop(0) if lst else p


_ConvState = collections.namedtuple('_ConvState', 'g relu has_bias c_in w_layout slot give_slot grad_dst uses')


def _conv_operands(x, weight, bias, stride, pad):
    xn = _pad_c4(to_nhwc(_f32c(x) if x.dim() != 4 else x.float()))
    wn = _pad_c4(to_nhwc(weight.float()))
    N, H, W, C = xn.shape
    K, R, S, _ = wn.shape
    g = _geom(N, H, W, C, K, R, S, stride, pad)
    y = torch.empty((N, g.P, g.Q, K), dtype=torch.float32, device=x.device)
    return xn, wn, (None if bias is None else _f32c(bias)), g, y


def _conv_state(x, weight, bias, g, relu, slot=None, give_slot=None):
    uses = getattr(weight, '_nnl_uses', None)
    if uses is not None:
        uses[0] += 1
    return _ConvState(g, relu, bias is not None, x.shape[1], (tuple(weight.shape), tuple(weight.stride())), slot, give_slot,
                      getattr(weight, '_nnl_grad_dst', None), uses)


def _with_k(g, K):
    return _geom(g.N, g.H, g.W, g.C, K, g.R, g.S, g.stride, g.pad)


def _conv_backward(st, xn, wn, y, dy, needs):
    if dy is None:
        return None, None, None
    g, K = st.g, st.g.K
    want_db = st.has_bias and needs[2]
    db = None
    pre = _padded_rows(dy, K) if (not st.relu and g.R == 1 and g.S == 1 and g.H == 1 and g.W == 1) else None
    if pre is not None and pre.shape[-1] != K:
        dy4 = pre
    else:
        dy4 = to_nhwc(dy.float())
        if st.relu:
            dy4, db = _conv_act_gate(y, dy4, g, st.relu, want_db)
        if K % 4 != 0:
            dy4 = _pad_c4(dy4)
    w4, g4 = wn, g
    if dy4.shape[-1] != K:
        w4, g4 = torch.nn.functional.pad(wn, (0, 0, 0, 0, 0, 0, 0, dy4.shape[-1] - K)), _with_k(g, dy4.shape[-1])
    dx = dw = None
    if needs[0]:
        dx = _conv_dgrad(st, dy4, w4, g4, K)
    elif st.slot is not None:
        st.slot.tensor, st.slot.closed = None, True
    if needs[1]:
        dw = _conv_wgrad(st, xn, dy4, g4, K)
    if db is None and want_db:
        db = _conv_bias_grad(dy4, g4, K)
    return dx, dw, db


def _conv_act_gate(y, dyn, g, relu, want_db):
    rows = g.N * g.P * g.Q
    gated = torch.empty_like(dyn)
    cb = int(lib.nnl_colsum_workspace_bytes(rows, g.K)) if want_db else 0
    cws = _workspace(cb, dyn.device, floor=True) if want_db else None
    db = torch.empty(g.K, dtype=torch.float32, device=dyn.device) if want_db else None
    check(lib.nnl_act_gate_colsum(ptr(dyn), ptr(y), ptr(gated), ptr(db), rows, g.K, int(relu), ptr(cws), cb, stream()))
    return gated, db


def _conv_dgrad_operands(dy4, w4, g4, K):
    ktail = g4.R == 1 and g4.S == 1 and g4.K % 4 == 0 and os.environ.get('NNL_IGEMM_KTAIL', '1') != '0'
    dyd, gd, padk, wkey = dy4, g4, 0, None
    if g4.K % 16 != 0 and g4.K >= 32 and not ktail:
        padk = 16 - g4.K % 16
        dyd, gd = torch.nn.functional.pad(dy4, (0, padk)), _with_k(g4, g4.K + padk)
        wkey = (w4.data_ptr(), tuple(w4.shape), padk)
        wt = _WT_PADDED.get(wkey) if _WT_ACTIVE else None
    else:
        wt = _WT_ACTIVE.get(w4.data_ptr()) if g4.K == K else None
        if wt is not None and tuple(wt.shape) != (g4.C, g4.R, g4.S, g4.K):
            wt = None
    if wt is None:
        wd = torch.nn.functional.pad(w4, (0, 0, 0, 0, 0, 0, 0, padk)) if padk else w4
        wt = torch.empty((gd.C, gd.R, gd.S, gd.K), dtype=torch.float32, device=dy4.device)
        check(lib.nnl_conv2d_weight_transpose(ptr(wd), ptr(wt), gd.K, gd.R, gd.S, gd.C, stream()))
        if wkey is not None and _WT_ACTIVE:
            _WT_PADDED[wkey] = wt
    return dyd, wt, gd


def _conv_dgrad(st, dy4, w4, g4, K):
    dyd, wt, g = _conv_dgrad_operands(dy4, w4, g4, K)
    dxn = torch.empty((g.N, g.H, g.W, g.C), dtype=torch.float32, device=dyd.device)
    wsb = int(lib.nnl_conv2d_dgrad_workspace_bytes(g))
    dws = _workspace(wsb, dyd.device)
    shortcut = None
    if st.slot is not None:
        shortcut, st.slot.tensor, st.slot.closed = st.slot.tensor, None, True
    fuse = shortcut is not None and g.K % 16 == 0 and g.R * g.S <= 49 and shortcut.numel() == dxn.numel() \
        and ((g.stride == 1 and (g.S <= 32 or g.pad <= 127)) or (g.stride == 2 and g.R == 3 and g.S == 3 and g.pad == 1))
    wmode = _wino_pref(w4.data_ptr() if g.K == K else 0, 1, g)
    u = _WINO_U_BWD.get((w4.data_ptr(), wmode)) if (wmode and g.K == K) else None
    if u is not None and u.numel() != _wino_u_numel(g.C, g.K, wmode):
        u = None
    check(lib.nnl_conv2d_dgrad_pre(ptr(dyd), ptr(wt), ptr(dxn), g, ptr(shortcut) if fuse else None, ptr(dws), wsb,
                                   ptr(_tile_counters(dyd.device) if wsb else None), ptr(u), stream()))
    if shortcut is not None and not fuse:
        dxn += shortcut.view_as(dxn)
    give = st.give_slot
    if give is not None and not give.closed and st.c_in == g.C:
        give.tensor = dxn
        return None
    return from_nhwc(dxn[..., :st.c_in] if st.c_in != g.C else dxn)


def _conv_wgrad(st, xn, dy4, g4, K):
    dst = st.grad_dst
    if dst is not None and st.uses is not None and st.uses[0] == 1 and dst.dim() == 4 and g4.K == K and st.c_in == g4.C \
            and dst.permute(0, 2, 3, 1).is_contiguous() and tuple(dst.shape) == (g4.K, g4.C, g4.R, g4.S):
        dwn = dst.permute(0, 2, 3, 1)
    else:
        dwn = torch.empty((g4.K, g4.R, g4.S, g4.C), dtype=torch.float32, device=dy4.device)
    wsb = int(lib.nnl_conv2d_wgrad_workspace_bytes(g4))
    ws = _workspace(wsb, dy4.device, floor=True)
    check(lib.nnl_conv2d_wgrad(ptr(xn), ptr(dy4), ptr(dwn), g4, ptr(ws), wsb, stream()))
    dw = from_nhwc(dwn[:K, :, :, :st.c_in])
    wshape, wstride = st.w_layout
    if (g4.R == 1 and g4.S == 1 and wshape == tuple(dw.shape) and wstride != tuple(dw.stride()) and dw.is_contiguous(memory_format=torch.channels_last)
            and wstride[1] == 1 and wstride[0] == dw.shape[1]):
        dw = dw.as_strided(wshape, wstride)
    return dw


def _conv_bias_grad(dy4, g4, K):
    rows = g4.N * g4.P * g4.Q
    db_full = torch.empty(g4.K, dtype=torch.float32, device=dy4.device)
    cb = int(lib.nnl_colsum_workspace_bytes(rows, g4.K))
    cws = _workspace(cb, dy4.device, floor=True)
    check(lib.nnl_colsum(ptr(dy4), ptr(db_full), rows, g4.K, ptr(cws), cb, stream()))
    return db_full[:K]


class _Conv2d(torch.autograd.Function):

    @staticmethod
    def forward(ctx, x, weight, bias, stride, pad, relu, slot=None, bn_pivot=None, give_slot=None):
        require_cuda(x, weight, bias)
        xn, wn, b, g, y = _conv_operands(x, weight, bias, stride, pad)
        N, K, C = g.N, g.K, g.C
        ctx.st = _conv_state(x, weight, bias, g, relu, slot, give_slot)
        wsb = int(lib.nnl_conv2d_fwd_workspace_bytes(g))
        ws = _workspace(wsb, x.device)
        part, rows = None, _lib.i32(0)
        if bn_pivot is not None:
            part = torch.empty(((N * g.P * g.Q + 63) // 64) * K * 2, dtype=torch.float32, device=x.device)
        wmode = _wino_pref(wn.data_ptr(), 0, g)
        u = _WINO_U_FWD.get((wn.data_ptr(), wmode)) if wmode else None
        if u is not None and u.numel() != _wino_u_numel(K, C, wmode):
            u = None
        check(lib.nnl_conv2d_fwd_pre(ptr(xn), ptr(wn), ptr(b), ptr(y), g, int(relu), ptr(ws), wsb, ptr(_tile_counters(x.device) if wsb else None),
                                     ptr(part), ptr(bn_pivot), ctypes.byref(rows) if part is not None else None, ptr(u), stream()))
        if part is None or rows.value == 0:
            part = torch.empty(0, dtype=torch.float32, device=x.device)
        else:
            part = part[:rows.value * K * 2]
        ctx.mark_non_differentiable(part)
        ctx.set_materialize_grads(False)
        ctx.save_for_backward(xn, wn, y if relu else None)
        return from_nhwc(y), part

    @staticmethod
    def backward(ctx, dy, _dpart=None):
        xn, wn, y = ctx.saved_tensors
        return _conv_backward(ctx.st, xn, wn, y, dy, ctx.needs_input_grad[:3]) + (None,) * 6


def _conv(x, weight, bias, *, stride=1, pad=0, relu=0, slot=None, bn_pivot=None, give_slot=None):
    return _Conv2d.apply(x, weight, bias, int(stride), int(pad), int(relu), slot, bn_pivot, give_slot)


def conv2d(x, weight, bias=None, stride=1, pad=0, relu=False, grad_slot=None, give_slot=None):
    return _conv(x, weight, bias, stride=stride, pad=pad, relu=relu, slot=grad_slot, give_slot=give_slot)[0]


class _ConvAddUp2(torch.autograd.Function):

    @staticmethod
    def forward(ctx, x, weight, bias, small, stride, pad):
        require_cuda(x, weight, bias, small)
        xn, wn, b, g, y = _conv_operands(x, weight, bias, stride, pad)
        sn = to_nhwc(small.float())
        ctx.small_shape = (g.N, g.P // 2, g.Q // 2, g.K)
        if tuple(sn.shape) != ctx.small_shape or g.P % 2 or g.Q % 2:
            raise _lib.NnlError('conv_add_upsampled: `small` %s is not [N, K, P/2, Q/2] of the %dx%d output' % (tuple(small.shape), g.P, g.Q))
        ctx.st = _conv_state(x, weight, bias, g, 0)
        check(lib.nnl_conv2d_fwd_add_up2(ptr(xn), ptr(wn), ptr(b), ptr(sn), ptr(y), g, stream()))
        ctx.save_for_backward(xn, wn)
        return from_nhwc(y)

    @staticmethod
    def backward(ctx, dy):
        dsmall = None
        if ctx.needs_input_grad[3]:
            dyn = to_nhwc(dy.float())
            N, h, w, K = ctx.small_shape
            ds = torch.empty(ctx.small_shape, dtype=torch.float32, device=dy.device)
            check(lib.nnl_upsample2_bwd(ptr(dyn), ptr(ds), N, h, w, K, stream()))
            dsmall = from_nhwc(ds)
        xn, wn = ctx.saved_tensors
        return _conv_backward(ctx.st, xn, wn, None, dy, ctx.needs_input_grad[:3]) + (dsmall, None, None)


def conv_add_upsampled(x, weight, bias, small, stride=1, pad=0):
    return _ConvAddUp2.apply(x, weight, bias, small, int(stride), int(pad))


def conv2d_with_bn_stats(x, weight, bias, stride, pad, bn_pivot, grad_slot=None, give_slot=None):
    return _conv(x, weight, bias, stride=stride, pad=pad, slot=grad_slot, bn_pivot=bn_pivot, give_slot=give_slot)


def _rows_in_place(x):
    return x.dtype == torch.float32 and x.dim() == 2 and x.stride(1) == 1 and x.stride(0) >= x.shape[1]


class _LinearSmall(torch.autograd.Function):

    @staticmethod
    def forward(ctx, x, weight, bias):
        require_cuda(x, weight, bias)
        x = x if _rows_in_place(x) else _f32c(x)
        w = _f32c(weight)
        b = None if bias is None else _f32c(bias)
        M, K = x.shape
        N = w.shape[0]
        y = torch.empty(M, N, dtype=torch.float32, device=x.device)
        check(lib.nnl_linear_small_fwd(ptr(x), ptr(w), ptr(b), ptr(y), M, K, x.stride(0) if M > 1 else K, N, stream()))
        ctx.save_for_backward(x, w)
        ctx.has_bias = bias is not None
        return y

    @staticmethod
    def backward(ctx, dy):
        x, w = ctx.saved_tensors
        M, K = x.shape
        N = w.shape[0]
        dy = _f32c(dy)
        dev = dy.device
        dx = torch.empty(M, K, dtype=torch.float32, device=dev) if ctx.needs_input_grad[0] else None
        dw = torch.empty(N, K, dtype=torch.float32, device=dev) if ctx.needs_input_grad[1] else None
        db = torch.empty(N, dtype=torch.float32, device=dev) if (ctx.has_bias and ctx.needs_input_grad[2]) else None
        wsb = int(lib.nnl_linear_small_bwd_workspace_bytes(M, K, N)) if (dw is not None or db is not None) else 0
        ws = _workspace(wsb, dev)
        check(lib.nnl_linear_small_bwd(ptr(dy), ptr(x), ptr(w), ptr(dx), ptr(dw), ptr(db), M, K, x.stride(0) if M > 1 else K, N, ptr(ws), wsb,
                                       stream()))
        return dx, dw, db


def linear(x, weight, bias=None, relu=False):
    lead = x.shape[:-1]
    x2 = x.reshape(-1, x.shape[-1])
    if not relu and weight.shape[0] <= 4 and x2.is_cuda and x2.shape[0] > 0:
        return _LinearSmall.apply(x2, weight, bias).reshape(*lead, weight.shape[0])
    y = _conv(x2[:, :, None, None], weight[:, :, None, None], bias, relu=relu)[0]
    return y.reshape(*lead, weight.shape[0])


def _rows_view(x):
    if x.dim() == 4:
        xn = to_nhwc(x.float())
        N, H, W, C = xn.shape
        return xn.view(-1, C), (lambda m: from_nhwc(m.view(N, H, W, C)))
    if x.dim() == 2:
        return _f32c(x), (lambda m: m)
    if x.dim() == 3:
        xn = x.float().permute(0, 2, 1).contiguous()
        N, L, C = xn.shape
        return xn.view(-1, C), (lambda m: m.view(N, L, C).permute(0, 2, 1))
    raise ValueError('bn_act: unsupported input rank %d' % x.dim())


def _relu_mask(rows, C, device):
    return torch.empty((rows * C + 31) // 32 + 2, dtype=torch.int32, device=device)


class _BNAct(torch.autograd.Function):
    @staticmethod
    def forward(ctx, x, residual, gamma, beta, running_mean, running_var, training, momentum, eps, relu, nbt, slot=None, ext=None,
                pivot_out=None):
        require_cuda(x, residual, gamma, beta)
        ctx.slot = slot
        xm, back = _rows_view(x)
        rows, C = xm.shape
        rm = None if residual is None else _rows_view(residual)[0]
        y = torch.empty_like(xm)
        mean = torch.empty(C, dtype=torch.float32, device=xm.device)
        invstd = torch.empty(C, dtype=torch.float32, device=xm.device)
        wsb = int(lib.nnl_bn_workspace_bytes(rows, C))
        ws = _workspace(wsb, xm.device)
        mask = _relu_mask(rows, C, xm.device) if relu else None
        check(lib.nnl_bn_fwd(ptr(xm), ptr(gamma), ptr(beta), ptr(rm), ptr(y), ptr(mean), ptr(invstd), ptr(running_mean),
                             ptr(running_var), rows, C, float(eps), float(momentum), int(training), int(relu), ptr(nbt),
                             ptr(mask), ptr(ext[0]) if ext else None, (ext[0].numel() // (2 * C)) if ext else 0,
                             ptr(ext[1]) if ext else None, ptr(pivot_out), ptr(ws), wsb, stream()))
        ctx.save_for_backward(xm, mask, gamma, mean, invstd)
        ctx.cfg = (training, relu, residual is not None, back)
        return back(y)

    @staticmethod
    def backward(ctx, dy):
        xm, mask, gamma, mean, invstd = ctx.saved_tensors
        training, relu, has_res, back = ctx.cfg
        dym = _rows_view(dy)[0]
        rows, C = xm.shape
        dx = torch.empty_like(xm)
        dres = torch.empty_like(xm) if (has_res and ctx.needs_input_grad[1]) else None
        dgamma = torch.empty(C, dtype=torch.float32, device=xm.device) if gamma is not None else None
        dbeta = torch.empty(C, dtype=torch.float32, device=xm.device) if gamma is not None else None
        wsb = int(lib.nnl_bn_workspace_bytes(rows, C))
        ws = _workspace(wsb, xm.device)
        check(lib.nnl_bn_bwd(ptr(dym), None, ptr(mask), ptr(xm), ptr(gamma), ptr(mean), ptr(invstd), ptr(dx), ptr(dres),
                             ptr(dgamma), ptr(dbeta), rows, C, int(training), int(relu), ptr(ws), wsb, stream()))
        if ctx.slot is not None and dres is not None:
            ctx.slot.tensor, dres = dres, None
        return (back(dx), None if dres is None else back(dres), dgamma, dbeta) + (None,) * 10


def _sync_group_size(group):
    import torch.distributed as dist
    return dist.get_world_size(group)


class _SyncBNAct(torch.autograd.Function):

    @staticmethod
    def forward(ctx, x, residual, gamma, beta, running_mean, running_var, momentum, eps, relu, nbt, group, comm, slot=None):
        require_cuda(x, residual, gamma, beta)
        ctx.slot = slot
        xm, back = _rows_view(x)
        rows, C = xm.shape
        rm = None if residual is None else _rows_view(residual)[0]
        dev = xm.device
        wsb = int(lib.nnl_bn_workspace_bytes(rows, C))
        ws = _workspace(wsb, dev)
        stats = torch.empty(2 * C + 2, dtype=torch.float32, device=dev)
        check(lib.nnl_bn_sync_stats(ptr(xm), ptr(stats), rows, C, ptr(ws), wsb, stream()))
        all_stats = comm.all_gather(stats, group)
        world = all_stats.shape[0]
        y = torch.empty_like(xm)
        mean = torch.empty(C, dtype=torch.float32, device=dev)
        invstd = torch.empty(C, dtype=torch.float32, device=dev)
        mask = _relu_mask(rows, C, dev) if relu else None
        check(lib.nnl_bn_sync_fwd(ptr(xm), ptr(all_stats), world, ptr(gamma), ptr(beta), ptr(rm), ptr(y), ptr(mean), ptr(invstd),
                                  ptr(running_mean), ptr(running_var), rows, C, float(eps), float(momentum), int(relu), ptr(nbt),
                                  ptr(mask), ptr(ws), wsb, stream()))
        ctx.save_for_backward(xm, mask, gamma, mean, invstd, all_stats)
        ctx.cfg = (relu, residual is not None, back, group, comm)
        return back(y)

    @staticmethod
    def backward(ctx, dy):
        xm, mask, gamma, mean, invstd, all_stats = ctx.saved_tensors
        relu, has_res, back, group, comm = ctx.cfg
        dym = _rows_view(dy)[0]
        rows, C = xm.shape
        dev = xm.device
        wsb = int(lib.nnl_bn_workspace_bytes(rows, C))
        ws = _workspace(wsb, dev)
        sums = torch.empty(2 * C, dtype=torch.float32, device=dev)
        check(lib.nnl_bn_sync_bwd_reduce(ptr(dym), None, ptr(mask), ptr(xm), ptr(mean), ptr(invstd), ptr(sums), rows, C, int(relu),
                                         ptr(ws), wsb, stream()))
        total = comm.all_reduce_sum(sums, group)
        dx = torch.empty_like(xm)
        dres = torch.empty_like(xm) if (has_res and ctx.needs_input_grad[1]) else None
        dgamma = torch.empty(C, dtype=torch.float32, device=dev) if gamma is not None else None
        dbeta = torch.empty(C, dtype=torch.float32, device=dev) if gamma is not None else None
        check(lib.nnl_bn_sync_bwd(ptr(dym), None, ptr(mask), ptr(xm), ptr(gamma), ptr(mean), ptr(invstd), ptr(sums), ptr(total),
                                  ptr(all_stats), int(all_stats.shape[0]), ptr(dx), ptr(dres), ptr(dgamma), ptr(dbeta), rows, C,
                                  int(relu), ptr(ws), wsb, stream()))
        if ctx.slot is not None and dres is not None:
            ctx.slot.tensor, dres = dres, None
        return (back(dx), None if dres is None else back(dres), dgamma, dbeta) + (None,) * 9


class DistComm:

    @staticmethod
    def all_gather(t, group):
        import torch.distributed as dist
        w = dist.get_world_size(group)
        out = torch.empty((w,) + tuple(t.shape), dtype=t.dtype, device=t.device)
        dist.all_gather(list(out.unbind(0)), t, group=group)
        return out

    @staticmethod
    def all_reduce_sum(t, group):
        import torch.distributed as dist
        out = t.clone()
        dist.all_reduce(out, op=dist.ReduceOp.SUM, group=group)
        return out


def _bn_mode(bn):
    training = bn.training or (bn.running_mean is None)
    momentum, nbt = 0.0, None
    if bn.training and bn.track_running_stats:
        nbt, momentum = bn.num_batches_tracked, bn.momentum
    stats = not training or bn.track_running_stats
    return training, momentum, nbt, (bn.running_mean if stats else None), (bn.running_var if stats else None)


def bn_act(bn, x, residual=None, relu=True, grad_slot=None, ext_stats=None, pivot_out=None):
    training, momentum, nbt, rmean, rvar = _bn_mode(bn)
    if momentum is None:
        nbt.add_(1)
        momentum, nbt = 1.0 / float(nbt.item()), None
    sync = getattr(bn, 'nnl_sync', None)
    if sync is not None and training:
        return _SyncBNAct.apply(x, residual, bn.weight, bn.bias, rmean, rvar, momentum, bn.eps, relu, nbt, sync[0], sync[1],
                                grad_slot)
    ext = ext_stats if (ext_stats is not None and training and ext_stats[0].numel() > 0) else None
    return _BNAct.apply(x, residual, bn.weight, bn.bias, rmean, rvar, training, momentum, bn.eps, relu, nbt, grad_slot, ext,
                        pivot_out if training else None)


class _ConcatPool(torch.autograd.Function):
    @staticmethod
    def forward(ctx, x):
        require_cuda(x)
        xn = to_nhwc(x.float())
        N, H, W, C = xn.shape
        out = torch.empty(N, 2 * C, dtype=torch.float32, device=x.device)
        am = torch.empty(N, C, dtype=torch.int32, device=x.device)
        check(lib.nnl_concat_pool_fwd(ptr(xn), ptr(out), ptr(am), N, H * W, C, stream()))
        ctx.save_for_backward(am)
        ctx.shape = (N, H, W, C)
        return out.view(N, 2 * C, 1, 1)

    @staticmethod
    def backward(ctx, dout):
        (am,) = ctx.saved_tensors
        N, H, W, C = ctx.shape
        dx = torch.empty(N, H, W, C, dtype=torch.float32, device=dout.device)
        check(lib.nnl_concat_pool_bwd(ptr(_f32c(dout.reshape(N, 2 * C))), ptr(am), ptr(dx), N, H * W, C, stream()))
        return from_nhwc(dx)


def conv_bn_act(conv, bn, x, residual=None, relu=True, conv_slot=None, bn_slot=None, conv_give=None):
    fuse = (bn.training and bn.track_running_stats and bn.running_mean is not None and bn.momentum is not None
            and getattr(bn, 'nnl_sync', None) is None and x.is_cuda and conv.bias is None and not conv.fuse_relu
            and torch.is_grad_enabled() and os.environ.get('NNL_BN_EPI_STATS', '1') != '0')

    def unfused(**kw):
        return bn_act(bn, conv(x, grad_slot=conv_slot, give_slot=conv_give), residual=residual, relu=relu, grad_slot=bn_slot, **kw)
    if not fuse:
        return unfused()
    pivot = getattr(bn, '_nnl_pivot', None)
    if pivot is None or pivot.device != x.device or pivot.numel() != bn.num_features:
        if torch.cuda.is_current_stream_capturing():
            return unfused()
        pivot = torch.empty(bn.num_features, dtype=torch.float32, device=x.device)
        object.__setattr__(bn, '_nnl_pivot', pivot)
        return unfused(pivot_out=pivot)
    y, part = conv2d_with_bn_stats(x, conv.weight, None, conv.stride[0], conv.padding[0], pivot, conv_slot, conv_give)
    return bn_act(bn, y, residual=residual, relu=relu, grad_slot=bn_slot, ext_stats=(part, pivot), pivot_out=pivot)


def linear_relu_bn(lin, bn, x):
    fuse = (bn.training and bn.track_running_stats and bn.running_mean is not None and bn.momentum is not None
            and getattr(bn, 'nnl_sync', None) is None and x.is_cuda and x.dim() == 2 and torch.is_grad_enabled()
            and os.environ.get('NNL_BN_EPI_STATS', '1') != '0')
    pivot = getattr(bn, '_nnl_pivot', None) if fuse else None
    if not fuse or pivot is None or pivot.device != x.device or pivot.numel() != bn.num_features:
        y = linear(x, lin.weight, lin.bias, relu=True)
        if not fuse or torch.cuda.is_current_stream_capturing():
            return bn_act(bn, y, relu=False)
        pivot = torch.empty(bn.num_features, dtype=torch.float32, device=x.device)
        object.__setattr__(bn, '_nnl_pivot', pivot)
        return bn_act(bn, y, relu=False, pivot_out=pivot)
    y, part = _conv(x[:, :, None, None], lin.weight[:, :, None, None], lin.bias, relu=1, bn_pivot=pivot)
    return bn_act(bn, y.reshape(x.shape[0], lin.weight.shape[0]), relu=False, ext_stats=(part, pivot), pivot_out=pivot)


def concat_pool2d(x):
    return _ConcatPool.apply(x)


class _MaxPool2d(torch.autograd.Function):
    @staticmethod
    def forward(ctx, x, ksize, stride, pad):
        require_cuda(x)
        xn = to_nhwc(x.float())
        N, H, W, C = xn.shape
        P, Q = (H + 2 * pad - ksize) // stride + 1, (W + 2 * pad - ksize) // stride + 1
        y = torch.empty(N, P, Q, C, dtype=torch.float32, device=x.device)
        idx = torch.empty(N, P, Q, C, dtype=torch.uint8, device=x.device)
        check(lib.nnl_maxpool2d_fwd(ptr(xn), ptr(y), ptr(idx), N, H, W, C, P, Q, ksize, stride, pad, stream()))
        ctx.save_for_backward(idx)
        ctx.cfg = (N, H, W, C, P, Q, ksize, stride, pad)
        return from_nhwc(y)

    @staticmethod
    def backward(ctx, dy):
        (idx,) = ctx.saved_tensors
        N, H, W, C, P, Q, ksize, stride, pad = ctx.cfg
        dyn = to_nhwc(dy.float())
        dx = torch.empty(N, H, W, C, dtype=torch.float32, device=dy.device)
        check(lib.nnl_maxpool2d_bwd(ptr(dyn), ptr(idx), ptr(dx), N, H, W, C, P, Q, ksize, stride, pad, stream()))
        return from_nhwc(dx), None, None, None


class _BNReLUMaxPool(torch.autograd.Function):

    @staticmethod
    def forward(ctx, x, gamma, beta, running_mean, running_var, training, momentum, eps, nbt, ksize, stride, pad):
        require_cuda(x, gamma, beta)
        xn = to_nhwc(x.float())
        N, H, W, C = xn.shape
        P, Q = (H + 2 * pad - ksize) // stride + 1, (W + 2 * pad - ksize) // stride + 1
        dev = x.device
        y = torch.empty(N, P, Q, C, dtype=torch.float32, device=dev)
        idx = torch.empty(N, P, Q, C, dtype=torch.uint8, device=dev)
        stats = torch.empty(4, C, dtype=torch.float32, device=dev)
        wsb = int(lib.nnl_bn_workspace_bytes(N * H * W, C))
        ws = _workspace(wsb, dev)
        check(lib.nnl_bn_relu_maxpool_fwd(ptr(xn), ptr(gamma), ptr(beta), ptr(y), ptr(idx), ptr(stats[0]), ptr(stats[1]),
                                          ptr(stats[2]), ptr(stats[3]), ptr(running_mean), ptr(running_var), N, H, W, C, P, Q,
                                          ksize, stride, pad, float(eps), float(momentum), int(training), ptr(nbt), ptr(ws), wsb,
                                          stream()))
        ctx.save_for_backward(xn, idx, gamma, beta, stats, y)
        ctx.cfg = (N, H, W, C, P, Q, ksize, stride, pad, training)
        return from_nhwc(y)

    @staticmethod
    def backward(ctx, dy):
        xn, idx, gamma, beta, stats, y = ctx.saved_tensors
        N, H, W, C, P, Q, ksize, stride, pad, training = ctx.cfg
        dyn = to_nhwc(dy.float())
        dx = torch.empty_like(xn)
        dgamma = torch.empty(C, dtype=torch.float32, device=xn.device) if gamma is not None else None
        dbeta = torch.empty(C, dtype=torch.float32, device=xn.device) if gamma is not None else None
        wsb = int(lib.nnl_bn_workspace_bytes(N * H * W, C))
        ws = _workspace(wsb, xn.device)
        check(lib.nnl_bn_relu_maxpool_bwd(ptr(dyn), ptr(y), ptr(idx), ptr(xn), ptr(gamma), ptr(beta), ptr(stats[0]), ptr(stats[1]),
                                          ptr(stats[2]), ptr(stats[3]), ptr(dx), ptr(dgamma), ptr(dbeta), N, H, W, C, P, Q, ksize, stride, pad,
                                          int(training), ptr(ws), wsb, stream()))
        return (from_nhwc(dx), dgamma, dbeta) + (None,) * 9


def conv_bn_relu_maxpool(conv, bn, pool, x):
    k, s, p = pool.kernel_size, pool.stride, pool.padding
    fuse = (x.is_cuda and isinstance(pool, torch.nn.MaxPool2d) and all(isinstance(v, int) for v in (k, s, p))
            and pool.dilation == 1 and not pool.ceil_mode and not pool.return_indices and 2 * p <= k and k * k <= 255
            and not (bn.training and getattr(bn, 'nnl_sync', None) is not None)
            and (bn.running_mean is not None or bn.training)
            and not (bn.training and bn.track_running_stats and bn.momentum is None)
            and bool(lib.nnl_bn_relu_maxpool_supported(bn.num_features)))
    if not fuse:
        return pool(conv_bn_act(conv, bn, x, relu=True))
    y = conv(x)
    training, momentum, nbt, rmean, rvar = _bn_mode(bn)
    return _BNReLUMaxPool.apply(y, bn.weight, bn.bias, rmean, rvar, training, momentum, bn.eps, nbt, k, s, p)


def maxpool2d(x, ksize=3, stride=2, pad=1):
    return _MaxPool2d.apply(x, int(ksize), int(stride), int(pad))


class TabularPlan:

    def __init__(self, weights):
        dev = weights[0].device
        self.key = tuple((w.data_ptr(), tuple(w.shape)) for w in weights) + (str(dev),)
        self.sync = None
        card = [int(w.shape[0]) for w in weights]
        dim = [int(w.shape[1]) for w in weights]
        self.ncat, self.cat_width, self.total_rows = len(weights), sum(dim), sum(card)
        col_off = np.concatenate([[0], np.cumsum(dim)[:-1]]).astype(np.int32)
        row_off = np.concatenate([[0], np.cumsum(card)[:-1]]).astype(np.int32)
        sizes = [c * d for c, d in zip(card, dim)]
        self.grad_sizes, self.shapes = sizes, [tuple(w.shape) for w in weights]
        grad_off = np.concatenate([[0], np.cumsum(sizes)[:-1]]).astype(np.int64)
        self.grad_elems = int(sum(sizes))
        t = lambda a, dt: torch.as_tensor(np.asarray(a), dtype=dt).to(dev)
        self.ptrs = t(np.array([w.data_ptr() for w in weights], dtype=np.int64), torch.int64)
        self.card, self.dim = t(card, torch.int32), t(dim, torch.int32)
        self.col_off, self.row_off, self.grad_off = t(col_off, torch.int32), t(row_off, torch.int32), t(grad_off, torch.int64)
        self.col_table = t(np.repeat(np.arange(self.ncat), dim), torch.int32)
        self.row_table = t(np.repeat(np.arange(self.ncat), card), torch.int32)
        self.flags = torch.zeros(self.total_rows, dtype=torch.int32, device=dev)
        self.max_dim = max(dim) if dim else 0
        blk_col, blk_first = [], []
        for j, n in enumerate(sizes):
            for f in range(0, n, 256):
                blk_col.append(j)
                blk_first.append(f)
        self.n_scan_blocks = len(blk_col)
        self.blk_col, self.blk_first = t(blk_col or [0], torch.int32), t(blk_first or [0], torch.int32)

    @staticmethod
    def for_weights(weights, cached=None):
        key = tuple((w.data_ptr(), tuple(w.shape)) for w in weights) + (str(weights[0].device),)
        return cached if (cached is not None and cached.key == key) else TabularPlan(weights)


class _TabEmbedConcat(torch.autograd.Function):

    @staticmethod
    def forward(ctx, xcat, cont, row_mask, cont_mask, plan, max_norm, *weights):
        require_cuda(xcat, cont, *weights)
        for w in weights:
            if not (w.is_contiguous() and w.dtype == torch.float32):
                raise _lib.NnlError('tab_embed_concat: embedding tables must be contiguous fp32 parameters')
        xcat = xcat.contiguous().long()
        bs = xcat.shape[0]
        n_cont = 0 if cont is None else cont.shape[1]
        cont = None if cont is None else _f32c(cont)
        row_mask = None if row_mask is None else _f32c(row_mask)
        cont_mask = None if cont_mask is None else _f32c(cont_mask)
        if max_norm is not None:
            if plan.sync is None:
                xren = xcat
            elif len(plan.sync) > 3 and plan.sync[3] is not None:
                xren = plan.sync[3]
            else:
                xren = _global_lookup_indices(xcat, plan.sync[:3])
            check(lib.nnl_tab_renorm(ptr(xren), ptr(plan.ptrs), ptr(plan.card), ptr(plan.dim), ptr(plan.row_off),
                                     ptr(plan.row_table), ptr(plan.flags), xren.shape[0], plan.ncat, plan.total_rows,
                                     float(max_norm), ptr(index_error_flag(xcat.device)), stream()))
        ld = plan.cat_width + n_cont
        out = torch.empty(bs, ld, dtype=torch.float32, device=xcat.device)
        check(lib.nnl_tab_gather_fwd(ptr(xcat), ptr(plan.ptrs), ptr(plan.card), ptr(plan.dim), ptr(plan.col_off),
                                     ptr(plan.col_table), ptr(row_mask), ptr(cont), ptr(cont_mask), ptr(out), bs, plan.ncat,
                                     plan.cat_width, n_cont, ld, stream()))
        ctx.save_for_backward(xcat, row_mask, cont_mask)
        ctx.plan, ctx.n_cont = plan, n_cont
        return out

    @staticmethod
    def backward(ctx, dout):
        xcat, row_mask, cont_mask = ctx.saved_tensors
        plan, n_cont = ctx.plan, ctx.n_cont
        bs = xcat.shape[0]
        flat = torch.empty(max(plan.grad_elems, 1), dtype=torch.float32, device=dout.device)
        dcont = torch.empty(bs, n_cont, dtype=torch.float32, device=dout.device) if (n_cont and ctx.needs_input_grad[1]) else None
        if plan.ncat and bs and 0 < plan.max_dim <= 32 and plan.grad_elems * bs <= (1 << 28) and os.environ.get('NNL_TAB_SCAN', '1') != '0':
            if not (dout.dtype == torch.float32 and dout.dim() == 2 and dout.stride(1) == 1 and dout.stride(0) >= dout.shape[1]):
                dout = _f32c(dout)
            check(lib.nnl_tab_scan_bwd(ptr(xcat), ptr(plan.card), ptr(plan.dim), ptr(plan.col_off), ptr(plan.grad_off), ptr(row_mask),
                                       ptr(cont_mask), ptr(dout), ptr(flat), ptr(dcont), ptr(plan.blk_col), ptr(plan.blk_first),
                                       plan.n_scan_blocks, plan.max_dim, bs, plan.ncat, plan.cat_width, n_cont, dout.stride(0), stream()))
        else:
            dout = _f32c(dout)
            wsb = int(lib.nnl_tab_scatter_bwd_workspace_bytes(bs, plan.ncat))
            ws = _workspace(wsb, dout.device, floor=True)
            check(lib.nnl_tab_scatter_bwd(ptr(xcat), ptr(plan.card), ptr(plan.dim), ptr(plan.col_off), ptr(plan.col_table),
                                          ptr(plan.grad_off), ptr(row_mask), ptr(cont_mask), ptr(dout), ptr(flat), plan.grad_elems,
                                          ptr(dcont), bs, plan.ncat, plan.cat_width, n_cont, dout.shape[1], ptr(ws), wsb, stream()))
        grads, o = [], 0
        for n, shp in zip(plan.grad_sizes, plan.shapes):
            grads.append(flat[o:o + n].view(shp))
            o += n
        return (None, dcont, None, None, None, None) + tuple(grads)


def _global_lookup_indices(xcat, sync):
    group, comm, cap = sync[:3]
    bs, ncat = xcat.shape
    if bs > cap:
        raise _lib.NnlError(f'tab_embed_concat: local batch {bs} exceeds the data-parallel capacity {cap}')
    pad = torch.zeros(cap + 1, ncat, dtype=torch.int64, device=xcat.device)
    pad[:bs] = xcat
    pad[cap, 0] = bs
    g = comm.all_gather(pad, group)
    counts, rows = g[:, cap, 0], g[:, :cap]
    valid = torch.arange(cap, device=xcat.device)[None, :] < counts[:, None]
    flat = rows.reshape(-1, ncat)
    fill = flat[valid.reshape(-1).to(torch.uint8).argmax()]
    return torch.where(valid.reshape(-1, 1), flat, fill).contiguous()


def keep_masks(shape_a, keep_a, shape_b, keep_b, device):
    na = 0 if shape_a is None else int(torch.Size(shape_a).numel())
    nb = 0 if shape_b is None else int(torch.Size(shape_b).numel())
    u = torch.rand(na + nb, dtype=torch.float32, device=device)
    a = torch.empty(shape_a, dtype=torch.float32, device=device) if na else None
    b = torch.empty(shape_b, dtype=torch.float32, device=device) if nb else None
    check(lib.nnl_keep_masks(ptr(u), ptr(a), na, float(keep_a), ptr(b), nb, float(keep_b), stream()))
    return a, b


def tab_embed_concat(xcat, weights, row_mask=None, cont=None, cont_mask=None, max_norm=None, plan=None, sync=None):
    plan = TabularPlan.for_weights(weights, plan)
    plan.sync = sync
    return _TabEmbedConcat.apply(xcat, cont, row_mask, cont_mask, plan, max_norm, *weights), plan


def embedding_renorm_drop(x, weight, mask, max_norm):
    out, _ = tab_embed_concat(x.view(-1, 1), [weight], None if mask is None else mask.view(1, -1), None, None, max_norm)
    return out


class _RetinaLoss(torch.autograd.Function):

    @staticmethod
    def forward(ctx, anchors, reg, clas, boxes, cats, beta, alpha, gamma):
        require_cuda(anchors, reg, clas, boxes, cats)
        anchors, reg, clas, boxes = _f32c(anchors), _f32c(reg), _f32c(clas), _f32c(boxes)
        cats = cats.contiguous().long()
        bs, A, K = clas.shape
        M = boxes.shape[1]
        dev = clas.device
        state = torch.empty(bs, A, dtype=torch.int32, device=dev)
        npos = torch.empty(bs, dtype=torch.float32, device=dev)
        out = torch.empty(3, dtype=torch.float32, device=dev)
        wsb = int(lib.nnl_retina_loss_workspace_bytes(bs, A))
        ws = _workspace(wsb, dev, floor=True)
        check(lib.nnl_retina_loss_fwd(ptr(anchors), ptr(reg), ptr(clas), ptr(boxes), ptr(cats), ptr(state), ptr(npos), ptr(out),
                                      bs, A, K, M, float(beta), float(alpha), float(gamma), ptr(ws), wsb, stream()))
        ctx.save_for_backward(anchors, reg, clas, boxes, cats, state, npos)
        ctx.hyper = (float(beta), float(alpha), float(gamma))
        return out

    @staticmethod
    def backward(ctx, dout):
        anchors, reg, clas, boxes, cats, state, npos = ctx.saved_tensors
        beta, alpha, gamma = ctx.hyper
        bs, A, K = clas.shape
        gup = _f32c(dout)[0:1].contiguous()
        dreg, dclas = torch.empty_like(reg), torch.empty_like(clas)
        check(lib.nnl_retina_loss_bwd(ptr(anchors), ptr(reg), ptr(clas), ptr(boxes), ptr(cats), ptr(state), ptr(npos), ptr(gup),
                                      ptr(dreg), ptr(dclas), bs, A, K, boxes.shape[1], beta, alpha, gamma, stream()))
        return None, dreg, dclas, None, None, None, None, None


def retina_loss(anchors, reg, clas, boxes, cats, beta=0.5, alpha=0.25, gamma=2.0):
    return _RetinaLoss.apply(anchors, reg, clas, boxes, cats, beta, alpha, gamma)


from .ops_text import (lstm_layer, embedding_rowmask, softmax_cross_entropy, cross_entropy_nd, seq_activation_reg)
__all__ += ['lstm_layer', 'embedding_rowmask', 'softmax_cross_entropy', 'cross_entropy_nd', 'seq_activation_reg', 'conv_add_upsampled']
```

Measured before the change: 5538 images/s.

## Add dedicated MFMA stem 7x7 conv kernels with fused BN statistics

Adds a specialized 7x7 stride-2 3->64 stem convolution kernel, using MFMA 32x32x2 f32 with a persistent tile loop and prefetch, plus a matching weight-gradient kernel. Input grad is skipped because the image input does not require it. The forward kernel also emits per-block BN partial sums against a pivot, so the fused BN+ReLU+maxpool only runs a finalize step instead of a separate stats pass over the large stem output. On the first call, or during stream capture, no pivot exists yet and the generic conv path runs. This adds a new specialized code path that must handle both NCHW and channels_last strides.

Measured after the change: 5607 images/s, median of 6. No clear change (+1.3%).

```diff
diff --git a/include/nnl.h b/include/nnl.h
--- a/include/nnl.h
+++ b/include/nnl.h
@@ -93,6 +93,13 @@
 size_t nnl_conv2d_wgrad_workspace_bytes(const nnl_conv_geom_t* g);
 int nnl_conv2d_wgrad(const float* x, const float* dy, float* dw, const nnl_conv_geom_t* g, void* workspace,
                      size_t workspace_bytes, void* stream);
+int nnl_stem_conv_supported(const nnl_conv_geom_t* g);
+int64_t nnl_stem_conv_bn_rows(const nnl_conv_geom_t* g);
+int nnl_stem_conv_fwd(const float* x, const int64_t* x_strides, const float* w, const int64_t* w_strides, float* y,
+                      const nnl_conv_geom_t* g, float* bn_partials, const float* bn_pivot, int32_t* bn_rows, void* stream);
+size_t nnl_stem_conv_wgrad_workspace_bytes(const nnl_conv_geom_t* g);
+int nnl_stem_conv_wgrad(const float* x, const int64_t* x_strides, const float* dy, float* dw, const nnl_conv_geom_t* g,
+                        void* workspace, size_t workspace_bytes, void* stream);
 size_t nnl_colsum_workspace_bytes(int64_t rows, int64_t cols);
 int nnl_sum_tensors(const float* const* src, int n, float* out, int64_t numel, void* stream);
 int nnl_colsum(const float* a, float* out, int64_t rows, int64_t cols, void* workspace, size_t workspace_bytes,
@@ -118,6 +125,11 @@
                             int64_t N, int64_t H, int64_t W, int64_t C, int64_t P, int64_t Q, int ks, int stride, int pad, float eps,
                             float momentum, int training, int64_t* num_batches_tracked, void* workspace, size_t workspace_bytes,
                             void* stream);
+int nnl_bn_relu_maxpool_fwd_ext(const float* x, const float* gamma, const float* beta, float* y, uint8_t* idx, float* save_mean,
+                                float* save_invstd, float* save_scale, float* save_shift, float* running_mean, float* running_var,
+                                int64_t N, int64_t H, int64_t W, int64_t C, int64_t P, int64_t Q, int ks, int stride, int pad, float eps,
+                                float momentum, int training, int64_t* num_batches_tracked, const float* ext_partials, int64_t ext_rows,
+                                const float* ext_pivot, float* pivot_out, void* workspace, size_t workspace_bytes, void* stream);
 int nnl_bn_relu_maxpool_bwd(const float* dpool, const float* y, const uint8_t* idx, const float* x, const float* gamma,
                             const float* beta, const float* mean, const float* invstd, const float* scale, const float* shift,
                             float* dx, float* dgamma, float* dbeta,
diff --git a/neuralnetworklibrary_amd/_lib.py b/neuralnetworklibrary_amd/_lib.py
--- a/neuralnetworklibrary_amd/_lib.py
+++ b/neuralnetworklibrary_amd/_lib.py
@@ -59,6 +59,11 @@
     'nnl_conv2d_dgrad': (C.c_int, [c_p, c_p, c_p, C.POINTER(ConvGeom), c_p, c_p, sz, c_p, c_p]),
     'nnl_conv2d_wgrad_workspace_bytes': (sz, [C.POINTER(ConvGeom)]),
     'nnl_conv2d_wgrad': (C.c_int, [c_p, c_p, c_p, C.POINTER(ConvGeom), c_p, sz, c_p]),
+    'nnl_stem_conv_supported': (C.c_int, [C.POINTER(ConvGeom)]),
+    'nnl_stem_conv_bn_rows': (i64, [C.POINTER(ConvGeom)]),
+    'nnl_stem_conv_fwd': (C.c_int, [c_p, C.POINTER(i64), c_p, C.POINTER(i64), c_p, C.POINTER(ConvGeom), c_p, c_p, C.POINTER(i32), c_p]),
+    'nnl_stem_conv_wgrad_workspace_bytes': (sz, [C.POINTER(ConvGeom)]),
+    'nnl_stem_conv_wgrad': (C.c_int, [c_p, C.POINTER(i64), c_p, c_p, C.POINTER(ConvGeom), c_p, sz, c_p]),
     'nnl_colsum_workspace_bytes': (sz, [i64, i64]),
     'nnl_colsum': (C.c_int, [c_p, c_p, i64, i64, c_p, sz, c_p]),
     'nnl_relu_gate_colsum': (C.c_int, [c_p, c_p, c_p, c_p, i64, i64, c_p, sz, c_p]),
@@ -71,6 +76,8 @@
     'nnl_bn_relu_maxpool_supported': (C.c_int, [i64]),
     'nnl_bn_relu_maxpool_fwd': (C.c_int, [c_p, c_p, c_p, c_p, c_p, c_p, c_p, c_p, c_p, c_p, c_p, i64, i64, i64, i64, i64, i64,
                                           C.c_int, C.c_int, C.c_int, f32, f32, C.c_int, c_p, c_p, sz, c_p]),
+    'nnl_bn_relu_maxpool_fwd_ext': (C.c_int, [c_p, c_p, c_p, c_p, c_p, c_p, c_p, c_p, c_p, c_p, c_p, i64, i64, i64, i64, i64, i64,
+                                              C.c_int, C.c_int, C.c_int, f32, f32, C.c_int, c_p, c_p, i64, c_p, c_p, c_p, sz, c_p]),
     'nnl_bn_relu_maxpool_bwd': (C.c_int, [c_p, c_p, c_p, c_p, c_p, c_p, c_p, c_p, c_p, c_p, c_p, c_p, c_p, i64, i64, i64, i64, i64, i64,
                                           C.c_int, C.c_int, C.c_int, C.c_int, c_p, sz, c_p]),
     'nnl_concat_pool_fwd': (C.c_int, [c_p, c_p, c_p, i64, i64, i64, c_p]),
diff --git a/neuralnetworklibrary_amd/csrc/batchnorm.hip b/neuralnetworklibrary_amd/csrc/batchnorm.hip
--- a/neuralnetworklibrary_amd/csrc/batchnorm.hip
+++ b/neuralnetworklibrary_amd/csrc/batchnorm.hip
@@ -788,11 +788,13 @@
 
 extern "C" int nnl_bn_relu_maxpool_supported(int64_t C) { return bnpool_ok(C) ? 1 : 0; }
 
-extern "C" int nnl_bn_relu_maxpool_fwd(const float* x, const float* gamma, const float* beta, float* y, uint8_t* idx,
-                                       float* save_mean, float* save_invstd, float* save_scale, float* save_shift,
-                                       float* running_mean, float* running_var, int64_t N, int64_t H, int64_t W, int64_t C,
-                                       int64_t P, int64_t Q, int ks, int stride, int pad, float eps, float momentum, int training,
-                                       int64_t* num_batches_tracked, void* workspace, size_t workspace_bytes, void* stream) {
+extern "C" int nnl_bn_relu_maxpool_fwd_ext(const float* x, const float* gamma, const float* beta, float* y, uint8_t* idx,
+                                           float* save_mean, float* save_invstd, float* save_scale, float* save_shift,
+                                           float* running_mean, float* running_var, int64_t N, int64_t H, int64_t W, int64_t C,
+                                           int64_t P, int64_t Q, int ks, int stride, int pad, float eps, float momentum, int training,
+                                           int64_t* num_batches_tracked, const float* ext_partials, int64_t ext_rows,
+                                           const float* ext_pivot, float* pivot_out, void* workspace, size_t workspace_bytes,
+                                           void* stream) {
   const long rows = (long)N * H * W;
   NNL_CHECK_ARG(N > 0 && H > 0 && W > 0 && P > 0 && Q > 0 && ks > 0 && ks * ks <= 255 && stride > 0 && pad >= 0 && 2 * pad <= ks,
                 "bn_relu_maxpool_fwd: bad geometry");
@@ -809,13 +811,23 @@
   float* shift = save_shift;
   const long CG = C / 4;
   NnlProfScope prof(NNL_PROF_ELEMENTWISE, s, (double)rows * C * (training ? 8.0 : 4.0) + (double)N * P * Q * C * 5.0);
-  if (training) {
+  if (training && ext_partials != nullptr && ext_rows > 0 && ext_pivot != nullptr) {
+    if (ext_rows >= 1024)
+      hipLaunchKernelGGL(bn_finalize_kernel<256>, dim3((unsigned)C), dim3(256), 0, s, ext_pivot, ext_partials, (int)ext_rows, gamma, beta,
+                         save_mean, save_invstd, running_mean, running_var, scale, shift, rows, (int)C, eps, momentum,
+                         (long long*)num_batches_tracked, pivot_out);
+    else
+      hipLaunchKernelGGL(bn_finalize_kernel<kFinLanes>, dim3((unsigned)nnl_cdiv(C, 4)), dim3(256), 0, s, ext_pivot, ext_partials,
+                         (int)ext_rows, gamma, beta, save_mean, save_invstd, running_mean, running_var, scale, shift, rows, (int)C, eps,
+                         momentum, (long long*)num_batches_tracked, pivot_out);
+    NNL_CHECK_LAUNCH();
+  } else if (training) {
     const Shape sh = make_shape(rows, CG);
     hipLaunchKernelGGL(bn_stats_kernel<4>, dim3(sh.gx, sh.gy), dim3(kBlock), 0, s, x, part, rows, (int)C, sh.L);
     NNL_CHECK_LAUNCH();
     hipLaunchKernelGGL(bn_finalize_kernel<kFinLanes>, dim3((unsigned)nnl_cdiv(C, 4)), dim3(256), 0, s, x, part, sh.gx, gamma, beta,
                        save_mean, save_invstd, running_mean, running_var, scale, shift, rows, (int)C, eps, momentum,
-                       (long long*)num_batches_tracked, (float*)nullptr);
+                       (long long*)num_batches_tracked, pivot_out);
     NNL_CHECK_LAUNCH();
   } else {
     NNL_CHECK_HIP(hipMemcpyAsync(save_mean, running_mean, sizeof(float) * C, hipMemcpyDeviceToDevice, s));
@@ -828,6 +840,16 @@
                      (int)H, (int)W, (int)CG, (int)P, (int)Q, ks, stride, pad);
   NNL_CHECK_LAUNCH();
   return NNL_OK;
+}
+
+extern "C" int nnl_bn_relu_maxpool_fwd(const float* x, const float* gamma, const float* beta, float* y, uint8_t* idx,
+                                       float* save_mean, float* save_invstd, float* save_scale, float* save_shift,
+                                       float* running_mean, float* running_var, int64_t N, int64_t H, int64_t W, int64_t C,
+                                       int64_t P, int64_t Q, int ks, int stride, int pad, float eps, float momentum, int training,
+                                       int64_t* num_batches_tracked, void* workspace, size_t workspace_bytes, void* stream) {
+  return nnl_bn_relu_maxpool_fwd_ext(x, gamma, beta, y, idx, save_mean, save_invstd, save_scale, save_shift, running_mean, running_var, N, H, W,
+                                     C, P, Q, ks, stride, pad, eps, momentum, training, num_batches_tracked, nullptr, 0, nullptr, nullptr,
+                                     workspace, workspace_bytes, stream);
 }
 
 extern "C" int nnl_bn_relu_maxpool_bwd(const float* dpool, const float* y, const uint8_t* idx, const float* x, const float* gamma,
diff --git a/neuralnetworklibrary_amd/csrc/stem_conv.hip b/neuralnetworklibrary_amd/csrc/stem_conv.hip
--- /dev/null
+++ b/neuralnetworklibrary_amd/csrc/stem_conv.hip
@@ -0,0 +1,415 @@
+#include "nnl_common.h"
+
+namespace {
+
+typedef float f32x4 __attribute__((ext_vector_type(4)));
+typedef float f32x16 __attribute__((ext_vector_type(16)));
+
+constexpr int kK = 64;
+constexpr int kTP = 8, kTQ = 16;
+constexpr int kPR = 2 * kTP + 5, kPC = 2 * kTQ + 5;
+constexpr int kRS = 112;
+constexpr int kPatch = kPR * kRS;
+constexpr int kPatchElems = kPR * kPC * 3;
+constexpr int kThreads = 256;
+constexpr int kPre = (kPatchElems + kThreads - 1) / kThreads;
+constexpr int kSteps = 25 * 3;
+constexpr int kFilt = kSteps * 2 * kK;
+constexpr int kGroup = 5;
+constexpr int kFwdGrid = 768, kWgradSlabs = 512;
+constexpr int kSlots = 160;
+constexpr int kSlab = kSlots * kK;
+
+struct StemP {
+  const float* x; int sxn, sxc, sxh, sxw;
+  const float* w; int swk, swc, swr, sws;
+  float* y;
+  const float* dy;
+  float* slabs;
+  float* bn_part; const float* bn_pivot;
+  int N, H, W, P, Q, tilesY, tilesX, ntiles;
+};
+
+__device__ __forceinline__ void tile_coords(const StemP& p, int tile, int& n, int& ty, int& tx) {
+  tx = tile % p.tilesX;
+  const int t = tile / p.tilesX;
+  ty = t % p.tilesY;
+  n = t / p.tilesY;
+}
+
+struct PatchMap {
+  int goff[kPre], meta[kPre];
+  template <bool CL>
+  __device__ __forceinline__ void init(const StemP& p) {
+#pragma unroll
+    for (int i = 0; i < kPre; ++i) {
+      const int idx = (int)threadIdx.x + i * kThreads;
+      int c, ry, cx;
+      if (CL) { const int pix = idx / 3; c = idx - pix * 3; ry = pix / kPC; cx = pix - ry * kPC; }
+      else { c = idx / (kPR * kPC); const int rem = idx - c * (kPR * kPC); ry = rem / kPC; cx = rem - ry * kPC; }
+      goff[i] = c * p.sxc + ry * p.sxh + cx * p.sxw;
+      meta[i] = idx < kPatchElems ? (ry | (cx << 5) | ((ry * kRS + cx * 3 + c) << 11)) : -1;
+    }
+  }
+  __device__ __forceinline__ void fetch(const StemP& p, int tile, float (&pre)[kPre]) const {
+    int n, ty, tx;
+    tile_coords(p, tile, n, ty, tx);
+    const int iy0 = ty * (2 * kTP) - 3, ix0 = tx * (2 * kTQ) - 3;
+    const float* x0 = p.x + ((long)n * p.sxn + (long)iy0 * p.sxh + (long)ix0 * p.sxw);
+#pragma unroll
+    for (int i = 0; i < kPre; ++i) {
+      int m = meta[i];
+      asm volatile("" : "+v"(m));
+      const int iy = iy0 + (m & 31), ix = ix0 + ((m >> 5) & 63);
+      const bool ok = m >= 0 && iy >= 0 && iy < p.H && ix >= 0 && ix < p.W;
+      pre[i] = ok ? x0[goff[i]] : 0.f;
+    }
+  }
+  __device__ __forceinline__ void store(float* __restrict__ sP, const float (&pre)[kPre]) const {
+#pragma unroll
+    for (int i = 0; i < kPre; ++i) {
+      int m = meta[i];
+      asm volatile("" : "+v"(m));
+      if (m >= 0) sP[m >> 11] = pre[i];
+    }
+  }
+};
+
+template <int NV>
+__device__ __forceinline__ void halve(float (&v)[32], int lane) {
+  const bool up = (lane & NV) != 0;
+#pragma unroll
+  for (int i = 0; i < NV; ++i) {
+    const float send = up ? v[i] : v[i + NV];
+    const float keep = up ? v[i + NV] : v[i];
+    v[i] = keep + __shfl_xor(send, NV, 64);
+  }
+}
+__device__ __forceinline__ float lanes32_sum(float (&v)[32], int lane) {
+  halve<16>(v, lane); halve<8>(v, lane); halve<4>(v, lane); halve<2>(v, lane); halve<1>(v, lane);
+  return v[0];
+}
+
+struct StepOps {
+  float b[kGroup], a0[kGroup], a1[kGroup];
+  __device__ __forceinline__ void load(const float* pA, const float* pB, const float* pC, const float* fB, int g) {
+#pragma unroll
+    for (int i = 0; i < kGroup; ++i) {
+      const int step = g * kGroup + i, m = step / 3, c = step - 3 * m, r0 = (2 * m) / 7, s0 = 2 * m - 7 * r0;
+      const float* base = m == 24 ? pC : (s0 == 6 ? pB : pA);
+      b[i] = base[r0 * kRS + s0 * 3 + c];
+      a0[i] = fB[step * 2 * kK];
+      a1[i] = fB[step * 2 * kK + 32];
+    }
+  }
+};
+
+template <bool CL>
+__global__ __launch_bounds__(kThreads, 3) void stem_fwd_kernel(const StemP p) {
+  __shared__ __attribute__((aligned(16))) float sF[kFilt];
+  __shared__ __attribute__((aligned(16))) float sP[kPatch];
+  __shared__ __attribute__((aligned(16))) float sPiv[kK];
+  __shared__ float sRed[4][kK][2];
+  const int tid = threadIdx.x, lane = tid & 63, wave = tid >> 6, h = lane >> 5, li = lane & 31;
+
+  float pre[kPre];
+  PatchMap pm;
+  pm.init<CL>(p);
+  int tile = blockIdx.x;
+  pm.fetch(p, tile, pre);
+
+  const bool wcl = p.swc == 1;
+  for (int idx = tid; idx < kK * 147; idx += kThreads) {
+    const int n = idx / 147, rem = idx - n * 147;
+    int c, r, s;
+    if (wcl) { r = rem / 21; const int j = rem - r * 21; s = j / 3; c = j - s * 3; }
+    else { c = rem / 49; const int t = rem - c * 49; r = t / 7; s = t - r * 7; }
+    const int tap = r * 7 + s;
+    sF[(((tap >> 1) * 3 + c) * 2 + (tap & 1)) * kK + n] = p.w[n * p.swk + c * p.swc + r * p.swr + s * p.sws];
+  }
+  if (tid < 3 * kK) sF[((24 * 3 + (tid >> 6)) * 2 + 1) * kK + (tid & 63)] = 0.f;
+  if (tid < kPR) sP[tid * kRS + kRS - 1] = 0.f;
+  if (tid < kK) sPiv[tid] = p.bn_part ? p.bn_pivot[tid] : 0.f;
+
+  const int py = 2 * wave + (li >> 4), px = li & 15;
+  const float* pC = sP + (2 * py) * kRS + 6 * px;
+  const float* pA = pC + 3 * h;
+  const float* pB = pC + (kRS - 18) * h;
+  const float* fB = sF + h * kK + li;
+
+  while (tile < p.ntiles) {
+    pm.store(sP, pre);
+    __syncthreads();
+    const int next = tile + (int)gridDim.x;
+    if (next < p.ntiles) pm.fetch(p, next, pre);
+
+    f32x16 acc0 = {0.f}, acc1 = {0.f};
+    StepOps cur, nxt;
+    cur.load(pA, pB, pC, fB, 0);
+#pragma unroll
+    for (int g = 0; g < kSteps / kGroup; ++g) {
+      if (g + 1 < kSteps / kGroup) nxt.load(pA, pB, pC, fB, g + 1);
+      __builtin_amdgcn_sched_barrier(0);
+#pragma unroll
+      for (int i = 0; i < kGroup; ++i) {
+        acc0 = __builtin_amdgcn_mfma_f32_32x32x2f32(cur.a0[i], cur.b[i], acc0, 0, 0, 0);
+        acc1 = __builtin_amdgcn_mfma_f32_32x32x2f32(cur.a1[i], cur.b[i], acc1, 0, 0, 0);
+      }
+      __builtin_amdgcn_sched_barrier(0);
+      if (g + 1 < kSteps / kGroup) cur = nxt;
+    }
+
+    int n, ty, tx;
+    tile_coords(p, tile, n, ty, tx);
+    const int op = ty * kTP + py, oq = tx * kTQ + px;
+    const bool valid = op < p.P && oq < p.Q;
+    if (valid) {
+      float* yp = p.y + (((long)n * p.P + op) * p.Q + oq) * kK + 4 * h;
+#pragma unroll
+      for (int g = 0; g < 4; ++g) {
+        const f32x4 v0 = {acc0[4 * g], acc0[4 * g + 1], acc0[4 * g + 2], acc0[4 * g + 3]};
+        const f32x4 v1 = {acc1[4 * g], acc1[4 * g + 1], acc1[4 * g + 2], acc1[4 * g + 3]};
+        *reinterpret_cast<f32x4*>(yp + 8 * g) = v0;
+        *reinterpret_cast<f32x4*>(yp + 32 + 8 * g) = v1;
+      }
+    }
+    if (p.bn_part) {
+      float s12[2];
+#pragma unroll
+      for (int sq = 0; sq < 2; ++sq) {
+        float d[32];
+#pragma unroll
+        for (int g = 0; g < 4; ++g) {
+          const f32x4 pv0 = *reinterpret_cast<const f32x4*>(sPiv + 8 * g + 4 * h);
+          const f32x4 pv1 = *reinterpret_cast<const f32x4*>(sPiv + 32 + 8 * g + 4 * h);
+#pragma unroll
+          for (int e = 0; e < 4; ++e) {
+            const float a = valid ? acc0[4 * g + e] - pv0[e] : 0.f;
+            const float b = valid ? acc1[4 * g + e] - pv1[e] : 0.f;
+            d[4 * g + e] = sq ? a * a : a;
+            d[16 + 4 * g + e] = sq ? b * b : b;
+          }
+        }
+        s12[sq] = lanes32_sum(d, lane);
+      }
+      const float s1 = s12[0], s2 = s12[1];
+      const int ch = (li >> 4) * 32 + (li & 3) + 8 * ((li & 15) >> 2) + 4 * h;
+      sRed[wave][ch][0] = s1;
+      sRed[wave][ch][1] = s2;
+    }
+    __syncthreads();
+    if (p.bn_part && tid < kK) {
+      const float a = ((sRed[0][tid][0] + sRed[1][tid][0]) + sRed[2][tid][0]) + sRed[3][tid][0];
+      const float b = ((sRed[0][tid][1] + sRed[1][tid][1]) + sRed[2][tid][1]) + sRed[3][tid][1];
+      p.bn_part[((long)tile * kK + tid) * 2 + 0] = a;
+      p.bn_part[((long)tile * kK + tid) * 2 + 1] = b;
+    }
+    tile = next;
+  }
+}
+
+template <bool CL>
+__global__ __launch_bounds__(kThreads) void stem_wgrad_kernel(const StemP p) {
+  __shared__ __attribute__((aligned(16))) float smem[128 * kK + kPatch];
+  float* const sD = smem;
+  float* const sP = smem + 128 * kK;
+  const int tid = threadIdx.x, lane = tid & 63, wave = tid >> 6, h = lane >> 5, li = lane & 31;
+  const int ps = wave >> 1, mt = wave & 1;
+
+  float pre[kPre];
+  f32x4 dpre[8];
+  auto dy_fetch = [&](int tile) {
+    int n, ty, tx;
+    tile_coords(p, tile, n, ty, tx);
+#pragma unroll
+    for (int i = 0; i < 8; ++i) {
+      const int idx = tid + i * kThreads, pix = idx >> 4, c4 = idx & 15;
+      const int op = ty * kTP + (pix >> 4), oq = tx * kTQ + (pix & 15);
+      const f32x4 z = {0.f, 0.f, 0.f, 0.f};
+      dpre[i] = (op < p.P && oq < p.Q) ? *reinterpret_cast<const f32x4*>(p.dy + (((long)n * p.P + op) * p.Q + oq) * kK + c4 * 4) : z;
+    }
+  };
+  PatchMap pm;
+  pm.init<CL>(p);
+  int tile = blockIdx.x;
+  pm.fetch(p, tile, pre);
+  dy_fetch(tile);
+  if (tid < kPR) sP[tid * kRS + kRS - 1] = 0.f;
+
+  const float* aB = sD + (ps * 64 + h) * kK + mt * 32 + li;
+  const float* bB[5];
+#pragma unroll
+  for (int nt = 0; nt < 5; ++nt) {
+    int slot = nt * 32 + li;
+    slot = slot < 147 ? slot : 0;
+    const int r = slot / 21, j = slot - r * 21;
+    bB[nt] = sP + (8 * ps + r) * kRS + j + 6 * h;
+  }
+  f32x16 acc[5];
+#pragma unroll
+  for (int nt = 0; nt < 5; ++nt) acc[nt] = f32x16{0.f};
+
+  while (tile < p.ntiles) {
+    pm.store(sP, pre);
+#pragma unroll
+    for (int i = 0; i < 8; ++i) *reinterpret_cast<f32x4*>(sD + (tid + i * kThreads) * 4) = dpre[i];
+    __syncthreads();
+    const int next = tile + (int)gridDim.x;
+    if (next < p.ntiles) { pm.fetch(p, next, pre); dy_fetch(next); }
+    float a = aB[0], b[5];
+#pragma unroll
+    for (int nt = 0; nt < 5; ++nt) b[nt] = bB[nt][0];
+#pragma unroll
+    for (int s = 0; s < 32; ++s) {
+      float an = 0.f, bn[5] = {0.f, 0.f, 0.f, 0.f, 0.f};
+      if (s < 31) {
+        const int off = ((s + 1) >> 3) * 2 * kRS + 12 * ((s + 1) & 7);
+        an = aB[(s + 1) * 128];
+#pragma unroll
+        for (int nt = 0; nt < 5; ++nt) bn[nt] = bB[nt][off];
+      }
+      __builtin_amdgcn_sched_barrier(0);
+#pragma unroll
+      for (int nt = 0; nt < 5; ++nt) acc[nt] = __builtin_amdgcn_mfma_f32_32x32x2f32(a, b[nt], acc[nt], 0, 0, 0);
+      __builtin_amdgcn_sched_barrier(0);
+      a = an;
+#pragma unroll
+      for (int nt = 0; nt < 5; ++nt) b[nt] = bn[nt];
+    }
+    __syncthreads();
+    tile = next;
+  }
+
+  float* ex = smem + (mt * 64 + lane) * 80;
+  if (ps == 1) {
+#pragma unroll
+    for (int nt = 0; nt < 5; ++nt)
+#pragma unroll
+      for (int g = 0; g < 4; ++g)
+        *reinterpret_cast<f32x4*>(ex + nt * 16 + 4 * g) = f32x4{acc[nt][4 * g], acc[nt][4 * g + 1], acc[nt][4 * g + 2], acc[nt][4 * g + 3]};
+  }
+  __syncthreads();
+  if (ps == 0) {
+    float* slab = p.slabs + (long)blockIdx.x * kSlab;
+#pragma unroll
+    for (int nt = 0; nt < 5; ++nt)
+#pragma unroll
+      for (int g = 0; g < 4; ++g) {
+        const f32x4 o = *reinterpret_cast<const f32x4*>(ex + nt * 16 + 4 * g);
+        const f32x4 v = {acc[nt][4 * g] + o[0], acc[nt][4 * g + 1] + o[1], acc[nt][4 * g + 2] + o[2], acc[nt][4 * g + 3] + o[3]};
+        *reinterpret_cast<f32x4*>(slab + (nt * 32 + li) * kK + mt * 32 + 8 * g + 4 * h) = v;
+      }
+  }
+}
+
+__global__ __launch_bounds__(256) void stem_wgrad_finish_kernel(const float* __restrict__ slabs, int nslabs, float* __restrict__ dw) {
+  __shared__ float red[8][32];
+  const int oi = threadIdx.x & 31, sg = threadIdx.x >> 5;
+  const int o = blockIdx.x * 32 + oi;
+  const float* src = slabs + o;
+  float a = 0.f;
+  int s = sg;
+  for (; s + 56 < nslabs; s += 64) {
+    float v[8];
+#pragma unroll
+    for (int u = 0; u < 8; ++u) v[u] = src[(long)(s + 8 * u) * kSlab];
+#pragma unroll
+    for (int u = 0; u < 8; ++u) a += v[u];
+  }
+  for (; s < nslabs; s += 8) a += src[(long)s * kSlab];
+  red[sg][oi] = a;
+  __syncthreads();
+  if (sg == 0) {
+    float t = red[0][oi];
+#pragma unroll
+    for (int u = 1; u < 8; ++u) t += red[u][oi];
+    dw[(o & 63) * 147 + (o >> 6)] = t;
+  }
+}
+
+bool geom_ok(const nnl_conv_geom_t* g) {
+  if (!g) return false;
+  if (g->C != 3 || g->R != 7 || g->S != 7 || g->stride != 2 || g->pad != 3 || g->K != kK) return false;
+  if (g->N <= 0 || g->H <= 0 || g->W <= 0) return false;
+  if (g->P != (g->H + 6 - 7) / 2 + 1 || g->Q != (g->W + 6 - 7) / 2 + 1 || g->P <= 0 || g->Q <= 0) return false;
+  if ((long)g->N * g->H * g->W * 3 >= (1L << 31) || (long)g->N * g->P * g->Q * kK >= (1L << 31)) return false;
+  const long tiles = (long)g->N * nnl_cdiv(g->P, kTP) * nnl_cdiv(g->Q, kTQ);
+  return tiles < (1L << 24);
+}
+
+int layout_of(const int64_t* st, long a, long b) {
+  if (st[3] == 1 && st[2] == b && st[1] == a * b && st[0] == 3 * a * b) return 1;
+  if (st[1] == 1 && st[3] == 3 && st[2] == 3 * b && st[0] == 3 * a * b) return 2;
+  return 0;
+}
+
+void fill_geom(StemP& p, const nnl_conv_geom_t* g, const int64_t* xs) {
+  p.sxn = (int)xs[0]; p.sxc = (int)xs[1]; p.sxh = (int)xs[2]; p.sxw = (int)xs[3];
+  p.N = g->N; p.H = g->H; p.W = g->W; p.P = g->P; p.Q = g->Q;
+  p.tilesY = (int)nnl_cdiv(g->P, kTP); p.tilesX = (int)nnl_cdiv(g->Q, kTQ);
+  p.ntiles = p.N * p.tilesY * p.tilesX;
+}
+
+}
+
+extern "C" int nnl_stem_conv_supported(const nnl_conv_geom_t* g) { return geom_ok(g) ? 1 : 0; }
+
+extern "C" int64_t nnl_stem_conv_bn_rows(const nnl_conv_geom_t* g) {
+  return geom_ok(g) ? (int64_t)g->N * nnl_cdiv(g->P, kTP) * nnl_cdiv(g->Q, kTQ) : 0;
+}
+
+extern "C" int nnl_stem_conv_fwd(const float* x, const int64_t* x_strides, const float* w, const int64_t* w_strides, float* y,
+                                 const nnl_conv_geom_t* g, float* bn_partials, const float* bn_pivot, int32_t* bn_rows, void* stream) {
+  if (bn_rows) *bn_rows = 0;
+  NNL_CHECK_ARG(geom_ok(g), "stem_conv_fwd: unsupported geometry (3 -> 64 channels, 7x7, stride 2, pad 3 only)");
+  NNL_CHECK_ARG(x && w && y && x_strides && w_strides, "stem_conv_fwd: null pointer");
+  const int xl = layout_of(x_strides, g->H, g->W), wl = layout_of(w_strides, 7, 7);
+  NNL_CHECK_ARG(xl != 0, "stem_conv_fwd: the input is neither NCHW-contiguous nor channels_last");
+  NNL_CHECK_ARG(wl != 0, "stem_conv_fwd: the filter is neither [K,3,7,7]-contiguous nor channels_last");
+  hipStream_t s = (hipStream_t)stream;
+  StemP p = {};
+  fill_geom(p, g, x_strides);
+  p.x = x; p.w = w; p.y = y;
+  p.swk = (int)w_strides[0]; p.swc = (int)w_strides[1]; p.swr = (int)w_strides[2]; p.sws = (int)w_strides[3];
+  const bool stats = bn_partials && bn_pivot && bn_rows;
+  p.bn_part = stats ? bn_partials : nullptr; p.bn_pivot = bn_pivot;
+  const int grid = p.ntiles < kFwdGrid ? p.ntiles : kFwdGrid;
+  NnlProfScope prof(NNL_PROF_CONV_FWD, s, 2.0 * g->N * g->P * g->Q * kK * 147.0);
+  NNL_ROUTE("stem_fwd_kernel<%s>:%s@%d", xl == 2 ? "nhwc" : "nchw", stats ? "stats" : "plain", grid);
+  if (xl == 2) hipLaunchKernelGGL(stem_fwd_kernel<true>, dim3(grid), dim3(kThreads), 0, s, p);
+  else hipLaunchKernelGGL(stem_fwd_kernel<false>, dim3(grid), dim3(kThreads), 0, s, p);
+  NNL_CHECK_LAUNCH();
+  if (stats) *bn_rows = p.ntiles;
+  return NNL_OK;
+}
+
+extern "C" size_t nnl_stem_conv_wgrad_workspace_bytes(const nnl_conv_geom_t* g) {
+  if (!geom_ok(g)) return 0;
+  const long tiles = (long)g->N * nnl_cdiv(g->P, kTP) * nnl_cdiv(g->Q, kTQ);
+  return (size_t)(tiles < kWgradSlabs ? tiles : kWgradSlabs) * kSlab * sizeof(float);
+}
+
+extern "C" int nnl_stem_conv_wgrad(const float* x, const int64_t* x_strides, const float* dy, float* dw, const nnl_conv_geom_t* g,
+                                   void* workspace, size_t workspace_bytes, void* stream) {
+  NNL_CHECK_ARG(geom_ok(g), "stem_conv_wgrad: unsupported geometry (3 -> 64 channels, 7x7, stride 2, pad 3 only)");
+  NNL_CHECK_ARG(x && dy && dw && x_strides, "stem_conv_wgrad: null pointer");
+  const int xl = layout_of(x_strides, g->H, g->W);
+  NNL_CHECK_ARG(xl != 0, "stem_conv_wgrad: the input is neither NCHW-contiguous nor channels_last");
+  NNL_CHECK_ARG(((uintptr_t)dy & 15) == 0, "stem_conv_wgrad: dy must be 16-byte aligned");
+  if (workspace == nullptr || workspace_bytes < nnl_stem_conv_wgrad_workspace_bytes(g))
+    return nnl_set_error(NNL_ERR_WORKSPACE, "stem_conv_wgrad: workspace too small");
+  hipStream_t s = (hipStream_t)stream;
+  StemP p = {};
+  fill_geom(p, g, x_strides);
+  p.x = x; p.dy = dy; p.slabs = (float*)workspace;
+  const int grid = p.ntiles < kWgradSlabs ? p.ntiles : kWgradSlabs;
+  NnlProfScope prof(NNL_PROF_CONV_WGRAD, s, 2.0 * g->N * g->P * g->Q * kK * 147.0);
+  NNL_ROUTE("stem_wgrad_kernel<%s>:slabs@%d", xl == 2 ? "nhwc" : "nchw", grid);
+  if (xl == 2) hipLaunchKernelGGL(stem_wgrad_kernel<true>, dim3(grid), dim3(kThreads), 0, s, p);
+  else hipLaunchKernelGGL(stem_wgrad_kernel<false>, dim3(grid), dim3(kThreads), 0, s, p);
+  NNL_CHECK_LAUNCH();
+  NNL_ROUTE("stem_wgrad_finish_kernel");
+  hipLaunchKernelGGL(stem_wgrad_finish_kernel, dim3(147 * kK / 32), dim3(256), 0, s, (const float*)workspace, grid, dw);
+  NNL_CHECK_LAUNCH();
+  return NNL_OK;
+}
diff --git a/neuralnetworklibrary_amd/ops.py b/neuralnetworklibrary_amd/ops.py
--- a/neuralnetworklibrary_amd/ops.py
+++ b/neuralnetworklibrary_amd/ops.py
@@ -443,7 +443,7 @@
     return lst.pop(0) if lst else p
 
 
-_ConvState = collections.namedtuple('_ConvState', 'g relu has_bias c_in w_layout slot give_slot grad_dst uses')
+_ConvState = collections.namedtuple('_ConvState', 'g relu has_bias c_in w_layout slot give_slot grad_dst uses stem')
 
 
 def _conv_operands(x, weight, bias, stride, pad):
@@ -456,12 +456,33 @@
     return xn, wn, (None if bias is None else _f32c(bias)), g, y
 
 
-def _conv_state(x, weight, bias, g, relu, slot=None, give_slot=None):
+def _conv_state(x, weight, bias, g, relu, slot=None, give_slot=None, stem=None):
     uses = getattr(weight, '_nnl_uses', None)
     if uses is not None:
         uses[0] += 1
     return _ConvState(g, relu, bias is not None, x.shape[1], (tuple(weight.shape), tuple(weight.stride())), slot, give_slot,
-                      getattr(weight, '_nnl_grad_dst', None), uses)
+                      getattr(weight, '_nnl_grad_dst', None), uses, stem)
+
+
+def _dense_strides(t):
+    n, c, h, w = t.shape
+    if t.is_contiguous():
+        return (_lib.i64 * 4)(c * h * w, h * w, w, 1)
+    if t.is_contiguous(memory_format=torch.channels_last):
+        return (_lib.i64 * 4)(h * w * c, 1, w * c, c)
+    return None
+
+
+def _stem_route(x, weight, bias, stride, pad, relu):
+    if os.environ.get('NNL_STEM_CONV', '1') == '0' or bias is not None or relu or stride != 2 or pad != 3:
+        return None
+    if x.dim() != 4 or x.shape[1] != 3 or tuple(weight.shape) != (64, 3, 7, 7) or x.dtype != torch.float32 or weight.dtype != torch.float32:
+        return None
+    xs, ws = _dense_strides(x), _dense_strides(weight)
+    g = _geom(x.shape[0], x.shape[2], x.shape[3], 3, 64, 7, 7, 2, 3)
+    if xs is None or ws is None or not lib.nnl_stem_conv_supported(g):
+        return None
+    return g, xs, ws
 
 
 def _with_k(g, K):
@@ -561,9 +582,14 @@
         dwn = dst.permute(0, 2, 3, 1)
     else:
         dwn = torch.empty((g4.K, g4.R, g4.S, g4.C), dtype=torch.float32, device=dy4.device)
-    wsb = int(lib.nnl_conv2d_wgrad_workspace_bytes(g4))
-    ws = _workspace(wsb, dy4.device, floor=True)
-    check(lib.nnl_conv2d_wgrad(ptr(xn), ptr(dy4), ptr(dwn), g4, ptr(ws), wsb, stream()))
+    if st.stem is not None:
+        wsb = int(lib.nnl_stem_conv_wgrad_workspace_bytes(g4))
+        ws = _workspace(wsb, dy4.device, floor=True)
+        check(lib.nnl_stem_conv_wgrad(ptr(xn), st.stem, ptr(dy4), ptr(dwn), g4, ptr(ws), wsb, stream()))
+    else:
+        wsb = int(lib.nnl_conv2d_wgrad_workspace_bytes(g4))
+        ws = _workspace(wsb, dy4.device, floor=True)
+        check(lib.nnl_conv2d_wgrad(ptr(xn), ptr(dy4), ptr(dwn), g4, ptr(ws), wsb, stream()))
     dw = from_nhwc(dwn[:K, :, :, :st.c_in])
     wshape, wstride = st.w_layout
     if (g4.R == 1 and g4.S == 1 and wshape == tuple(dw.shape) and wstride != tuple(dw.stride()) and dw.is_contiguous(memory_format=torch.channels_last)
@@ -586,6 +612,9 @@
     @staticmethod
     def forward(ctx, x, weight, bias, stride, pad, relu, slot=None, bn_pivot=None, give_slot=None):
         require_cuda(x, weight, bias)
+        stem = None if ctx.needs_input_grad[0] else _stem_route(x, weight, bias, stride, pad, relu)
+        if stem is not None:
+            return _Conv2d._stem_forward(ctx, x, weight, stem, slot, bn_pivot, give_slot)
         xn, wn, b, g, y = _conv_operands(x, weight, bias, stride, pad)
         N, K, C = g.N, g.K, g.C
         ctx.st = _conv_state(x, weight, bias, g, relu, slot, give_slot)
@@ -607,6 +636,23 @@
         ctx.mark_non_differentiable(part)
         ctx.set_materialize_grads(False)
         ctx.save_for_backward(xn, wn, y if relu else None)
+        return from_nhwc(y), part
+
+    @staticmethod
+    def _stem_forward(ctx, x, weight, stem, slot, bn_pivot, give_slot):
+        g, xs, ws = stem
+        ctx.st = _conv_state(x, weight, None, g, 0, slot, give_slot, stem=xs)
+        y = torch.empty((g.N, g.P, g.Q, g.K), dtype=torch.float32, device=x.device)
+        part, rows = None, _lib.i32(0)
+        if bn_pivot is not None:
+            part = torch.empty(int(lib.nnl_stem_conv_bn_rows(g)) * g.K * 2, dtype=torch.float32, device=x.device)
+        check(lib.nnl_stem_conv_fwd(ptr(x), xs, ptr(weight), ws, ptr(y), g, ptr(part), ptr(bn_pivot),
+                                    ctypes.byref(rows) if part is not None else None, stream()))
+        if part is None or rows.value == 0:
+            part = torch.empty(0, dtype=torch.float32, device=x.device)
+        ctx.mark_non_differentiable(part)
+        ctx.set_materialize_grads(False)
+        ctx.save_for_backward(x, None, None)
         return from_nhwc(y), part
 
     @staticmethod
@@ -952,7 +998,7 @@
 class _BNReLUMaxPool(torch.autograd.Function):
 
     @staticmethod
-    def forward(ctx, x, gamma, beta, running_mean, running_var, training, momentum, eps, nbt, ksize, stride, pad):
+    def forward(ctx, x, gamma, beta, running_mean, running_var, training, momentum, eps, nbt, ksize, stride, pad, ext=None, pivot_out=None):
         require_cuda(x, gamma, beta)
         xn = to_nhwc(x.float())
         N, H, W, C = xn.shape
@@ -963,10 +1009,11 @@
         stats = torch.empty(4, C, dtype=torch.float32, device=dev)
         wsb = int(lib.nnl_bn_workspace_bytes(N * H * W, C))
         ws = _workspace(wsb, dev)
-        check(lib.nnl_bn_relu_maxpool_fwd(ptr(xn), ptr(gamma), ptr(beta), ptr(y), ptr(idx), ptr(stats[0]), ptr(stats[1]),
-                                          ptr(stats[2]), ptr(stats[3]), ptr(running_mean), ptr(running_var), N, H, W, C, P, Q,
-                                          ksize, stride, pad, float(eps), float(momentum), int(training), ptr(nbt), ptr(ws), wsb,
-                                          stream()))
+        check(lib.nnl_bn_relu_maxpool_fwd_ext(ptr(xn), ptr(gamma), ptr(beta), ptr(y), ptr(idx), ptr(stats[0]), ptr(stats[1]),
+                                              ptr(stats[2]), ptr(stats[3]), ptr(running_mean), ptr(running_var), N, H, W, C, P, Q,
+                                              ksize, stride, pad, float(eps), float(momentum), int(training), ptr(nbt),
+                                              ptr(ext[0]) if ext else None, (ext[0].numel() // (2 * C)) if ext else 0,
+                                              ptr(ext[1]) if ext else None, ptr(pivot_out), ptr(ws), wsb, stream()))
         ctx.save_for_backward(xn, idx, gamma, beta, stats, y)
         ctx.cfg = (N, H, W, C, P, Q, ksize, stride, pad, training)
         return from_nhwc(y)
@@ -984,7 +1031,7 @@
         check(lib.nnl_bn_relu_maxpool_bwd(ptr(dyn), ptr(y), ptr(idx), ptr(xn), ptr(gamma), ptr(beta), ptr(stats[0]), ptr(stats[1]),
                                           ptr(stats[2]), ptr(stats[3]), ptr(dx), ptr(dgamma), ptr(dbeta), N, H, W, C, P, Q, ksize, stride, pad,
                                           int(training), ptr(ws), wsb, stream()))
-        return (from_nhwc(dx), dgamma, dbeta) + (None,) * 9
+        return (from_nhwc(dx), dgamma, dbeta) + (None,) * 11
 
 
 def conv_bn_relu_maxpool(conv, bn, pool, x):
@@ -997,9 +1044,27 @@
             and bool(lib.nnl_bn_relu_maxpool_supported(bn.num_features)))
     if not fuse:
         return pool(conv_bn_act(conv, bn, x, relu=True))
-    y = conv(x)
     training, momentum, nbt, rmean, rvar = _bn_mode(bn)
-    return _BNReLUMaxPool.apply(y, bn.weight, bn.bias, rmean, rvar, training, momentum, bn.eps, nbt, k, s, p)
+    stats = (isinstance(conv, torch.nn.Conv2d) and bn.training and bn.track_running_stats and bn.running_mean is not None
+             and bn.momentum is not None and conv.bias is None
+             and not getattr(conv, 'fuse_relu', False)
+             and torch.is_grad_enabled() and os.environ.get('NNL_BN_EPI_STATS', '1') != '0' and not x.requires_grad
+             and conv.dilation == (1, 1) and conv.groups == 1 and conv.stride == (2, 2) and conv.padding == (3, 3) and conv.padding_mode == 'zeros'
+             and _stem_route(x, conv.weight, None, 2, 3, 0) is not None)
+    y = ext = pivot = None
+    if stats:
+        pivot = getattr(bn, '_nnl_pivot', None)
+        if pivot is not None and pivot.device == x.device and pivot.numel() == bn.num_features:
+            y, part = conv2d_with_bn_stats(x, conv.weight, None, 2, 3, pivot)
+            ext = (part, pivot) if part.numel() > 0 else None
+        elif torch.cuda.is_current_stream_capturing():
+            pivot = None
+        else:
+            pivot = torch.empty(bn.num_features, dtype=torch.float32, device=x.device)
+            object.__setattr__(bn, '_nnl_pivot', pivot)
+    if y is None:
+        y = conv(x)
+    return _BNReLUMaxPool.apply(y, bn.weight, bn.bias, rmean, rvar, training, momentum, bn.eps, nbt, k, s, p, ext, pivot)
 
 
 def maxpool2d(x, ksize=3, stride=2, pad=1):
```
